# huj31415/nbody3d-webgpu

Hardware: AMD Instinct MI355X
Metric: pair-interactions/s (higher is better)
Workload: dtype f32; 1 GPU; N=262144 Plummer sphere, dt=1e-3, G=1, eps2=1e-4, i-sharded over 1 GPU(s); n=262144, kernel_variant=f32pk_symw_ipl16_j1_w2048_r32t128, parallelism=1gpu

## Files before the change

include/nbody3d_hip.h:

```cpp
#ifndef NBODY3D_HIP_H
#define NBODY3D_HIP_H

#include <stddef.h>
#include <stdint.h>

#ifdef __cplusplus
extern "C" {
#endif
#if defined(__GNUC__)
#pragma GCC visibility push(default)
#endif

#define NB_ABI_VERSION 2u
#define NB_ABI_MINOR 4u

typedef struct nb_sim nb_sim;

typedef enum nb_status {
    NB_OK = 0,
    NB_ERR_INVALID = 1,
    NB_ERR_NO_DEVICE = 2,
    NB_ERR_HIP = 3,
    NB_ERR_STATE = 4,
    NB_ERR_NOMEM = 5,
    NB_ERR_COMM = 6,
    NB_NOT_READY = 7
} nb_status;

typedef enum nb_precision { NB_F32 = 0, NB_F64 = 1 } nb_precision;

#define NB_FLAG_EXT_STREAM 1u
#define NB_FLAG_LDS_ONLY 4u
#define NB_FLAG_NO_FUSE 8u
#define NB_FLAG_POISON 16u

#define NB_FLAG_JPK_FENCED 32u

#define NB_FLAG_NO_SYM 64u

#define NB_FLAG_SYM_SHARD 128u

#define NB_FLAG_WHOLE_SWEEPS 256u

#define NB_FLAG_SINGLE_SWEEPS 512u

typedef enum nb_array { NB_BODIES = 0, NB_VEL = 1, NB_ACCEL = 2, NB_JERK = 3  } nb_array;

typedef enum nb_integrator { NB_INT_LEAPFROG = 0, NB_INT_HERMITE4 = 1 } nb_integrator;

typedef struct nb_config {
    uint32_t struct_size;
    uint32_t n;
    uint32_t precision;
    uint32_t tile;
    double eps2;
    int32_t device;
    uint32_t shard_begin;
    uint32_t shard_count;
    void *ext_stream;
    void *ext_bodies;
    uint32_t force_variant;
    uint32_t jsplit;
    uint32_t flags;
    uint32_t layer_budget_mib;
    uint32_t integrator;
    uint32_t reserved[3];
} nb_config;

uint32_t nb_abi_version(void);
uint32_t nb_abi_minor(void);

int nb_device_count(void);

int nb_create(const nb_config *cfg, nb_sim **out);

void nb_destroy(nb_sim *s);

int nb_upload(nb_sim *s, const void *bodies, const void *vel, const void *accel);

int nb_set_params(nb_sim *s, double dt, double G);

int nb_step(nb_sim *s, uint32_t nsteps);

int nb_download(nb_sim *s, void *bodies, void *vel, void *accel);

int nb_sync(nb_sim *s);

const char *nb_last_error(nb_sim *s);


int nb_device_ptr(nb_sim *s, int which , void **out);

typedef int (*nb_exchange_fn)(void *user, void *bodies_dev, size_t elem_size,
                              uint32_t n, uint32_t shard_begin,
                              uint32_t shard_count, void *hip_stream);
int nb_set_exchange(nb_sim *s, nb_exchange_fn fn, void *user);

typedef int (*nb_exchange_wait_fn)(void *user, void *hip_stream);
int nb_set_exchange_overlapped(nb_sim *s, nb_exchange_fn begin, nb_exchange_wait_fn wait, void *user);

#define NB_RCCL_ID_BYTES 128
#define NB_RCCL_OVERLAP 1u
int nb_rccl_unique_id(void *id_out );
int nb_rccl_attach(nb_sim *s, const void *id, int nranks, int rank, uint32_t flags);
int nb_rccl_detach(nb_sim *s);
int nb_rccl_info(nb_sim *s, int *nranks, int *rank, int *rccl_version);

typedef struct nb_multi nb_multi;
int nb_multi_create(const nb_config *cfg, uint32_t n_shards, const int32_t *devices, nb_multi **out);
void nb_multi_destroy(nb_multi *m);
int nb_multi_upload(nb_multi *m, const void *bodies, const void *vel, const void *accel);
int nb_multi_set_params(nb_multi *m, double dt, double G);
int nb_multi_step(nb_multi *m, uint32_t nsteps);
int nb_multi_download(nb_multi *m, void *bodies, void *vel, void *accel);
int nb_multi_sync(nb_multi *m);
const char *nb_multi_last_error(nb_multi *m);
int nb_multi_diagnostics(nb_multi *m, double out[5]);
const char *nb_multi_variant_name(nb_multi *m);
typedef enum nb_multi_collective { NB_MULTI_PEER = 0, NB_MULTI_RCCL = 1, NB_MULTI_PEER_OVERLAP = 2 } nb_multi_collective;
int nb_multi_set_collective(nb_multi *m, int mode );
int nb_multi_collective_info(nb_multi *m, int *mode, int *nranks, int *rccl_version);


int nb_enable_timing(nb_sim *s, int on);
int nb_kernel_times(nb_sim *s, double *force_ms, double *integrate_ms,
                    uint32_t *launches);
int nb_step_times(nb_sim *s, double *force_ms, double *integrate_ms, double *exchange_ms,
                  uint32_t *launches);
typedef struct nb_step_timing {
    uint32_t struct_size;
    uint32_t launches;
    double force_ms;
    double sym_reduce_ms;
    double reduce_scatter_ms;
    double integrate_ms;
    double allgather_ms;
    double span_ms;
    uint32_t reduce_scatters;
    uint32_t allgathers;
} nb_step_timing;
int nb_step_times2(nb_sim *s, nb_step_timing *out);
int nb_integrate_pass(nb_sim *s, uint32_t reps, double *avg_ms);
int nb_force_pass(nb_sim *s, uint32_t reps, double *avg_ms);

const char *nb_variant_name(nb_sim *s);

int nb_shape_info(nb_sim *s, uint32_t *jsplit, uint32_t *j_per_split, uint32_t *own_split0,
                  uint32_t *own_splits);



int nb_download_jerk(nb_sim *s, void *jerk);

int nb_upload_derivs(nb_sim *s, const void *accel, const void *jerk);

#define NB_BLOCK_FROZEN 1u
typedef struct nb_block_steps {
    uint32_t struct_size;
    uint32_t max_level;
    uint32_t min_level;
    uint32_t flags;
    double   eta;
} nb_block_steps;
int nb_set_block_steps(nb_sim *s, const nb_block_steps *cfg );

struct nb_block_stats {
    uint32_t struct_size, enabled;
    uint64_t outer_steps, block_steps, body_steps;
    uint64_t clamped;
    uint32_t finest_level, reserved;
};
int nb_block_stats(nb_sim *s, struct nb_block_stats *out, int reset);
int nb_download_levels(nb_sim *s, uint8_t *levels );
int nb_upload_levels(nb_sim *s, const uint8_t *levels );

int nb_frame_request(nb_sim *s);
int nb_frame_acquire(nb_sim *s, int wait, const float **bodies, const float **speed,
                     uint64_t *step_index);


int nb_diagnostics(nb_sim *s, double out[5]);

#define NB_FIELD_AT_BODIES 1u
#define NB_FIELD_F64       2u
#define NB_FIELD_DEVICE    4u
typedef struct nb_field_request {
    uint32_t struct_size;
    uint32_t m;
    uint32_t flags;
    uint32_t first_body;
    const void *points;
    void *accel;
    void *phi;
} nb_field_request;
int nb_field_eval(nb_sim *s, const nb_field_request *req);
int nb_multi_field_eval(nb_multi *m, const nb_field_request *req);

#define NB_NBR_AT_BODIES 1u
#define NB_NBR_DEVICE    4u
typedef struct nb_neighbor_request {
    uint32_t struct_size;
    uint32_t m;
    uint32_t flags;
    uint32_t first_body;
    const void *points;
    const void *radii;
    double radius;
    uint32_t *index;
    void *dist2;
    uint32_t *count;
} nb_neighbor_request;
int nb_neighbors(nb_sim *s, const nb_neighbor_request *req);
int nb_multi_neighbors(nb_multi *m, const nb_neighbor_request *req);
int nb_neighbors_shape(nb_sim *s, uint32_t m, uint32_t *batch, uint32_t *chunks, uint32_t *j_per_chunk);

#if defined(__GNUC__)
#pragma GCC visibility pop
#endif
#ifdef __cplusplus
}
#endif
#endif
```

nbody3d-webgpu_amd/csrc/kernels/symmetric.hip.h:

```cpp
#pragma once

namespace nb {

template <typename T> struct SymRowT { T x, y, z; };
using SymRow = SymRowT<float>;

constexpr uint32_t kFlushSteps = 4096;

template <int NG>
__device__ __forceinline__ void flush_resident_sums(float (*hi)[64], const int lane, const bool flushed, nb_f2 (&ax)[NG], nb_f2 (&ay)[NG], nb_f2 (&az)[NG])
{
    if (flushed) {
#pragma unroll
        for (int c = 0; c < NG; ++c) {
            hi[6 * c + 0][lane] += ax[c].x; hi[6 * c + 1][lane] += ay[c].x; hi[6 * c + 2][lane] += az[c].x;
            hi[6 * c + 3][lane] += ax[c].y; hi[6 * c + 4][lane] += ay[c].y; hi[6 * c + 5][lane] += az[c].y;
        }
    } else {
#pragma unroll
        for (int c = 0; c < NG; ++c) {
            hi[6 * c + 0][lane] = ax[c].x; hi[6 * c + 1][lane] = ay[c].x; hi[6 * c + 2][lane] = az[c].x;
            hi[6 * c + 3][lane] = ax[c].y; hi[6 * c + 4][lane] = ay[c].y; hi[6 * c + 5][lane] = az[c].y;
        }
    }
// ... 90 lines not shown
#pragma unroll
                    for (int c = 0; c < 4; ++c) r[c] = r[c] * d2[c];
#pragma unroll
                    for (int c = 0; c < 4; ++c) r[c] = nb_f2{nb_rsq(r[c].x), nb_rsq(r[c].y)};
#pragma unroll
                    for (int c = 0; c < 4; ++c) si[c] = pm * r[c];
#pragma unroll
                    for (int c = 0; c < 4; ++c) sj[c] = mi[c0g + c] * r[c];
#pragma unroll
                    for (int c = 0; c < 4; ++c) ax[c0g + c] = __builtin_elementwise_fma(si[c], dx[c], ax[c0g + c]);
#pragma unroll
                    for (int c = 0; c < 4; ++c) ay[c0g + c] = __builtin_elementwise_fma(si[c], dy[c], ay[c0g + c]);
#pragma unroll
                    for (int c = 0; c < 4; ++c) az[c0g + c] = __builtin_elementwise_fma(si[c], dz[c], az[c0g + c]);
#pragma unroll
                    for (int c = 0; c < 4; ++c) bx[u] = __builtin_elementwise_fma(-sj[c], dx[c], bx[u]);
#pragma unroll
                    for (int c = 0; c < 4; ++c) by[u] = __builtin_elementwise_fma(-sj[c], dy[c], by[u]);
#pragma unroll
                    for (int c = 0; c < 4; ++c) bz[u] = __builtin_elementwise_fma(-sj[c], dz[c], bz[u]);
                }
            }
#pragma unroll
            for (int u = 0; u < J; ++u) {
                tx[u] = wave_rot1(tx[u]); ty[u] = wave_rot1(ty[u]); tz[u] = wave_rot1(tz[u]); tm[u] = wave_rot1(tm[u]);
                bx[u] = nb_f2{wave_rot1(bx[u].x), wave_rot1(bx[u].y)};
                by[u] = nb_f2{wave_rot1(by[u].x), wave_rot1(by[u].y)};
                bz[u] = nb_f2{wave_rot1(bz[u].x), wave_rot1(bz[u].y)};
            }
        }
        if (sym) {
            SymRow* out = partial + (size_t)(pl.t_layer0 + d) * pl.np + tstart + lane;
            if constexpr (WS == 1) {
#pragma unroll
                for (int u = 0; u < J; ++u) out[u * 64] = SymRow{bx[u].x + bx[u].y, by[u].x + by[u].y, bz[u].x + bz[u].y};
            } else {
                const int buf = done++ & 1;
#pragma unroll
                for (int u = 0; u < J; ++u) {
                    red[buf][w][3 * u + 0][lane] = bx[u].x + bx[u].y;
                    red[buf][w][3 * u + 1][lane] = by[u].x + by[u].y;
                    red[buf][w][3 * u + 2][lane] = bz[u].x + bz[u].y;
                }
                __syncthreads();
                if (w == done % WS) {
#pragma unroll
                    for (int u = 0; u < J; ++u) {
                        float sx = red[buf][0][3 * u + 0][lane], sy = red[buf][0][3 * u + 1][lane], sz = red[buf][0][3 * u + 2][lane];
#pragma unroll
                        for (int ww = 1; ww < WS; ++ww) { sx += red[buf][ww][3 * u + 0][lane]; sy += red[buf][ww][3 * u + 1][lane]; sz += red[buf][ww][3 * u + 2][lane]; }
                        out[u * 64] = SymRow{sx, sy, sz};
                    }
                }
            }
        }
    }
    SymRow* out = partial + (size_t)(pl.r_layer0 + q) * pl.np + (size_t)g * S + w * RB + lane;
#pragma unroll
    for (int c = 0; c < NG; ++c) {
        out[(2 * c) * 64] = SymRow{ax[c].x, ay[c].x, az[c].x};
        out[(2 * c + 1) * 64] = SymRow{ax[c].y, ay[c].y, az[c].y};
    }
}

struct SymWK { uint32_t np, nsb, W, total_hi, total_lo, n_hi, zc, ups, r_layer0, t_layer0; };
#define SYMW_PLAN_PARAMS const uint32_t W_, const uint32_t ups_, const uint32_t nsb_, const uint32_t zc_, const uint32_t r_layer0_, const uint32_t t_layer0_
typedef uint32_t nb_u4 __attribute__((ext_vector_type(4)));
template <int TAIL>
__device__ __forceinline__ void symw_record_and_tail(const uint32_t* rec_at, nb_u4& rec, uint32_t (&tail)[TAIL])
{
    static_assert(TAIL == 1 || TAIL == 4, "f32: eps2; f64: G, eps2");
    constexpr int kTailOffset = 4 * 8 + 6 * 4;
    if constexpr (TAIL == 1) {
        asm volatile("s_load_dwordx4 %0, %2, 0x0\n\ts_load_dword %1, %3, %4\n\ts_waitcnt lgkmcnt(0)"
                     : "=&s"(rec), "=&s"(tail[0]) : "s"(rec_at), "s"(__builtin_amdgcn_kernarg_segment_ptr()), "n"(kTailOffset) : "memory");
    } else {
        nb_u4 t;
        asm volatile("s_load_dwordx4 %0, %2, 0x0\n\ts_load_dwordx4 %1, %3, %4\n\ts_waitcnt lgkmcnt(0)"
                     : "=&s"(rec), "=&s"(t) : "s"(rec_at), "s"(__builtin_amdgcn_kernarg_segment_ptr()), "n"(kTailOffset) : "memory");
        tail[0] = t.x; tail[1] = t.y; tail[2] = t.z; tail[3] = t.w;
    }
}

__device__ __forceinline__ SymWK symw_plan_words(uint32_t S, uint32_t cps, uint32_t W, uint32_t ups, uint32_t nsb, uint32_t zc, uint32_t r_layer0, uint32_t t_layer0)
{
    const uint32_t H = (nsb - 1u) >> 1, n_hi = (nsb & 1u) ? 0u : nsb >> 1;
    const uint32_t total_lo = (H + 1u) * cps + zc, total_hi = total_lo + (n_hi ? cps : 0u);
    return SymWK{(nsb + (zc ? 1u : 0u)) * S, nsb, W, total_hi, total_lo, n_hi, zc, ups, r_layer0, t_layer0};
}

template <int NG, int J, bool PAIR>
__device__ __forceinline__ void symw_sweeps(const uint32_t* __restrict__ gtab, const float4* __restrict__ bodies, SymRow* __restrict__ partial, SymRow* __restrict__ spill,
                                            SYMW_PLAN_PARAMS, uint32_t* __restrict__ queue, const uint32_t npieces, const uint32_t pieces_off)
{
    static_assert(!PAIR || J == 1, "paired sweeps: one traveler per lane and sweep");
    constexpr uint32_t S = 128u * NG;
    constexpr int GW = NG < 4 ? NG : 4;
    constexpr uint32_t CH = 64u * J;
    constexpr uint32_t CPS = S / CH;
    const SymWK pl = symw_plan_words(S, CPS, W_, ups_, nsb_, zc_, r_layer0_, t_layer0_);
    const int lane = threadIdx.x & 63, wi = threadIdx.x >> 6;
    const uint32_t w = __builtin_amdgcn_readfirstlane(blockIdx.x * 4u + wi);
    const bool active = w < pl.W;
    NB_STAMP(0);
    __shared__ float red[4][6 * NG][64];
    __shared__ uint32_t fin[4];
    const uint32_t ups = pl.ups, ush = (uint32_t)__builtin_ctz(ups), ustep = 64u >> ush,
                   tab1 = 2u * (pl.np / S);
    nb_u4 rec;
    uint32_t tail[1];
    symw_record_and_tail(gtab + tab1 + 4u * (active ? w : 0u), rec, tail);
    const float eps2 = __builtin_bit_cast(float, tail[0]);
    const nb_f2 e2 = nb_f2{eps2, eps2};
    const uint32_t first_lo = pl.n_hi * pl.total_hi, first_z = first_lo + (pl.nsb - pl.n_hi) * pl.total_lo;
    const uint32_t slot = rec.w;
    NB_STAMP_LIGHT(1);
    bool first_part = true;

    auto run = [&](uint32_t u, const uint32_t uend, const uint32_t piece_layer) -> uint32_t {
        uint32_t gfin = ~0u;
        while (u < uend) {
            const uint32_t p = u >> ush;
            uint32_t g, k, total;
            if (p < first_lo) { g = p / pl.total_hi; k = p - g * pl.total_hi; total = pl.total_hi; }
            else if (p < first_z) { const uint32_t r = p - first_lo; g = pl.n_hi + r / pl.total_lo; k = r - (g - pl.n_hi) * pl.total_lo; total = pl.total_lo; }
            else { g = pl.nsb; k = p - first_z; total = pl.zc; }
            const uint32_t ring = g < pl.nsb ? total - CPS - pl.zc : 0u;
            const uint32_t both_end = g < pl.nsb ? ring + pl.zc : 0u;
            uint32_t ug_end = (p - k + total) * ups;
            if (ug_end > uend) ug_end = uend;

            nb_f2 xi[NG], yi[NG], zi[NG], mi[NG], ax[NG], ay[NG], az[NG];
            {
                const float4* rb = bodies + (size_t)g * S + lane;
#pragma unroll
                for (int c = 0; c < NG; ++c) {
                    const float4 b0 = ld4(rb + (2 * c) * 64), b1 = ld4(rb + (2 * c + 1) * 64);
                    xi[c] = nb_f2{b0.x, b1.x}; yi[c] = nb_f2{b0.y, b1.y}; zi[c] = nb_f2{b0.z, b1.z}; mi[c] = nb_f2{b0.w, b1.w};
                    ax[c] = nb_f2{0, 0}; ay[c] = nb_f2{0, 0}; az[c] = nb_f2{0, 0};
                }
            }
            uint32_t since = 0;
            bool flushed = false;
            while (u < ug_end) {
                const uint32_t q0 = u & (ups - 1u);
                bool pair = false;
                if constexpr (PAIR) pair = q0 == 0u && ug_end - u >= 2u * ups && k + 1u < both_end;
                uint32_t nun = ups - q0;
                if (nun > ug_end - u) nun = ug_end - u;
                const uint32_t s0 = q0 * ustep, s1 = s0 + nun * ustep;
                u += pair ? 2u * ups : nun;
                if (since >= kFlushSteps) {
                    flush_resident_sums<NG>(red[wi], lane, flushed, ax, ay, az);
                    flushed = true;
                    since = 0;
                }
                since += pair ? 128u : s1 - s0;
                const bool sym = k < both_end, zsweep = k >= ring && sym;
                const uint32_t d = k / CPS;
                uint32_t tb = g + 1 + d;
                if (tb >= pl.nsb) tb -= pl.nsb;
                const uint32_t tstart = k < ring ? tb * S + (k % CPS) * CH : zsweep ? pl.nsb * S + (k - ring) * CH : g * S + (k - both_end) * CH;
                const uint32_t zrow = g * pl.zc + (k - ring);
                ++k;
                if constexpr (PAIR) {
                    if (pair) {
                        const bool zsweep1 = k >= ring;
                        const uint32_t d1 = k / CPS;
                        uint32_t tb1 = g + 1 + d1;
                        if (tb1 >= pl.nsb) tb1 -= pl.nsb;
                        const uint32_t tstart1 = zsweep1 ? pl.nsb * S + (k - ring) * CH : tb1 * S + (k % CPS) * CH;
                        const uint32_t zrow1 = g * pl.zc + (k - ring);
                        ++k;
                        const float4 t0 = ld4(bodies + tstart + lane), t1 = ld4(bodies + tstart1 + lane);
                        nb_f2 tx = nb_f2{t0.x, t1.x}, ty = nb_f2{t0.y, t1.y}, tz = nb_f2{t0.z, t1.z}, tm = nb_f2{t0.w, t1.w};
                        float bx0 = 0, bx1 = 0, by0 = 0, by1 = 0, bz0 = 0, bz1 = 0;
                        if (first_part) NB_STAMP(2);
                        for (uint32_t st = 0; st < 64u; ++st) {
                            nb_f2 sx = nb_f2{0, 0}, sy = nb_f2{0, 0}, sz = nb_f2{0, 0};
#pragma unroll
                            for (int c0g = 0; c0g < NG; c0g += GW) {
#pragma unroll
                                for (int f = 0; f < 2; ++f) {
                                    nb_f2 dx[GW], dy[GW], dz[GW], d2[GW], r[GW], si[GW], sj[GW];
#pragma unroll
                                    for (int c = 0; c < GW; ++c) dx[c] = symw_sub(f, tx, xi[c0g + c]);
#pragma unroll
                                    for (int c = 0; c < GW; ++c) dy[c] = symw_sub(f, ty, yi[c0g + c]);
#pragma unroll
                                    for (int c = 0; c < GW; ++c) dz[c] = symw_sub(f, tz, zi[c0g + c]);
#pragma unroll
                                    for (int c = 0; c < GW; ++c) d2[c] = __builtin_elementwise_fma(dx[c], dx[c], e2);
#pragma unroll
                                    for (int c = 0; c < GW; ++c) d2[c] = __builtin_elementwise_fma(dy[c], dy[c], d2[c]);
#pragma unroll
                                    for (int c = 0; c < GW; ++c) d2[c] = __builtin_elementwise_fma(dz[c], dz[c], d2[c]);
#pragma unroll
                                    for (int c = 0; c < GW; ++c) r[c] = d2[c] * d2[c];
#pragma unroll
                                    for (int c = 0; c < GW; ++c) r[c] = r[c] * d2[c];
#pragma unroll
                                    for (int c = 0; c < GW; ++c) r[c] = nb_f2{nb_rsq(r[c].x), nb_rsq(r[c].y)};
#pragma unroll
                                    for (int c = 0; c < GW; ++c) si[c] = symw_mul(f, tm, r[c]);
#pragma unroll
                                    for (int c = 0; c < GW; ++c) sj[c] = mi[c0g + c] * r[c];
#pragma unroll
                                    for (int c = 0; c < GW; ++c) ax[c0g + c] = __builtin_elementwise_fma(si[c], dx[c], ax[c0g + c]);
#pragma unroll
                                    for (int c = 0; c < GW; ++c) ay[c0g + c] = __builtin_elementwise_fma(si[c], dy[c], ay[c0g + c]);
#pragma unroll
                                    for (int c = 0; c < GW; ++c) az[c0g + c] = __builtin_elementwise_fma(si[c], dz[c], az[c0g + c]);
#pragma unroll
                                    for (int c = 0; c < GW; ++c) sx = symw_fnma(f, sj[c], dx[c], sx);
#pragma unroll
                                    for (int c = 0; c < GW; ++c) sy = symw_fnma(f, sj[c], dy[c], sy);
#pragma unroll
                                    for (int c = 0; c < GW; ++c) sz = symw_fnma(f, sj[c], dz[c], sz);
                                }
                            }
                            tx = nb_f2{wave_rot1(tx.x), wave_rot1(tx.y)}; ty = nb_f2{wave_rot1(ty.x), wave_rot1(ty.y)};
                            tz = nb_f2{wave_rot1(tz.x), wave_rot1(tz.y)}; tm = nb_f2{wave_rot1(tm.x), wave_rot1(tm.y)};
                            wave_rot1_add(bx0, sx.x); wave_rot1_add(bx1, sx.y); wave_rot1_add(by0, sy.x); wave_rot1_add(by1, sy.y);
                            wave_rot1_add(bz0, sz.x); wave_rot1_add(bz1, sz.y);
                            __builtin_amdgcn_sched_barrier(0);
                        }
                        if (first_part) { NB_STAMP_LIGHT(3); first_part = false; }
                        const uint32_t home = ((uint32_t)lane + 1u) & 63u;
                        SymRow* out0 = (zsweep ? spill + (size_t)zrow * CH : partial + (size_t)(pl.t_layer0 + d) * pl.np + tstart) + home;
                        SymRow* out1 = (zsweep1 ? spill + (size_t)zrow1 * CH : partial + (size_t)(pl.t_layer0 + d1) * pl.np + tstart1) + home;
                        *out0 = SymRow{bx0, by0, bz0};
                        *out1 = SymRow{bx1, by1, bz1};
                        continue;
                    }
                }
                float tx[J], ty[J], tz[J], tm[J];
                nb_f2 bx[J], by[J], bz[J];
                const uint32_t src = ((uint32_t)lane - s0) & 63u;
#pragma unroll
                for (int uu = 0; uu < J; ++uu) {
                    const float4 t = ld4(bodies + tstart + uu * 64 + src);
                    tx[uu] = t.x; ty[uu] = t.y; tz[uu] = t.z; tm[uu] = t.w;
                    bx[uu] = nb_f2{0, 0}; by[uu] = nb_f2{0, 0}; bz[uu] = nb_f2{0, 0};
                }
                auto steps = [&](auto both) {
                    constexpr bool BOTH = decltype(both)::value;
                    for (uint32_t st = s0; st < s1; ++st) {
#pragma unroll
                        for (int uu = 0; uu < J; ++uu) {
                            const nb_f2 px = nb_f2{tx[uu], tx[uu]}, py = nb_f2{ty[uu], ty[uu]}, pz = nb_f2{tz[uu], tz[uu]}, pm = nb_f2{tm[uu], tm[uu]};
#pragma unroll
                            for (int c0g = 0; c0g < NG; c0g += GW) {
                                nb_f2 dx[GW], dy[GW], dz[GW], d2[GW], r[GW], si[GW], sj[GW];
#pragma unroll
                                for (int c = 0; c < GW; ++c) dx[c] = px - xi[c0g + c];
#pragma unroll
                                for (int c = 0; c < GW; ++c) dy[c] = py - yi[c0g + c];
#pragma unroll
                                for (int c = 0; c < GW; ++c) dz[c] = pz - zi[c0g + c];
#pragma unroll
                                for (int c = 0; c < GW; ++c) d2[c] = __builtin_elementwise_fma(dx[c], dx[c], e2);
#pragma unroll
                                for (int c = 0; c < GW; ++c) d2[c] = __builtin_elementwise_fma(dy[c], dy[c], d2[c]);
#pragma unroll
                                for (int c = 0; c < GW; ++c) d2[c] = __builtin_elementwise_fma(dz[c], dz[c], d2[c]);
#pragma unroll
                                for (int c = 0; c < GW; ++c) r[c] = d2[c] * d2[c];
#pragma unroll
                                for (int c = 0; c < GW; ++c) r[c] = r[c] * d2[c];
#pragma unroll
                                for (int c = 0; c < GW; ++c) r[c] = nb_f2{nb_rsq(r[c].x), nb_rsq(r[c].y)};
#pragma unroll
                                for (int c = 0; c < GW; ++c) si[c] = pm * r[c];
                                if constexpr (BOTH) {
#pragma unroll
                                    for (int c = 0; c < GW; ++c) sj[c] = mi[c0g + c] * r[c];
                                }
#pragma unroll
                                for (int c = 0; c < GW; ++c) ax[c0g + c] = __builtin_elementwise_fma(si[c], dx[c], ax[c0g + c]);
#pragma unroll
                                for (int c = 0; c < GW; ++c) ay[c0g + c] = __builtin_elementwise_fma(si[c], dy[c], ay[c0g + c]);
#pragma unroll
                                for (int c = 0; c < GW; ++c) az[c0g + c] = __builtin_elementwise_fma(si[c], dz[c], az[c0g + c]);
                                if constexpr (BOTH) {
#pragma unroll
                                    for (int c = 0; c < GW; ++c) bx[uu] = __builtin_elementwise_fma(-sj[c], dx[c], bx[uu]);
#pragma unroll
                                    for (int c = 0; c < GW; ++c) by[uu] = __builtin_elementwise_fma(-sj[c], dy[c], by[uu]);
#pragma unroll
                                    for (int c = 0; c < GW; ++c) bz[uu] = __builtin_elementwise_fma(-sj[c], dz[c], bz[uu]);
                                }
                            }
                        }
#pragma unroll
                        for (int uu = 0; uu < J; ++uu) {
                            tx[uu] = wave_rot1(tx[uu]); ty[uu] = wave_rot1(ty[uu]); tz[uu] = wave_rot1(tz[uu]); tm[uu] = wave_rot1(tm[uu]);
                            if constexpr (BOTH) {
                                bx[uu] = nb_f2{wave_rot1(bx[uu].x), wave_rot1(bx[uu].y)};
                                by[uu] = nb_f2{wave_rot1(by[uu].x), wave_rot1(by[uu].y)};
                                bz[uu] = nb_f2{wave_rot1(bz[uu].x), wave_rot1(bz[uu].y)};
                            }
                        }
                    }
                };
                if (first_part) NB_STAMP(2);
                if (sym) steps(std::true_type{}); else steps(std::false_type{});
                if (first_part) { NB_STAMP_LIGHT(3); first_part = false; }
                if (sym) {
                    SymRow* out = (s0 != 0 ? spill + (size_t)slot * CH : zsweep ? spill + (size_t)zrow * CH : partial + (size_t)(pl.t_layer0 + d) * pl.np + tstart)
                                  + (((uint32_t)lane - s1) & 63u);
#pragma unroll
                    for (int uu = 0; uu < J; ++uu) out[uu * 64] = SymRow{bx[uu].x + bx[uu].y, by[uu].x + by[uu].y, bz[uu].x + bz[uu].y};
                }
            }
            if (u >= uend && piece_layer != ~0u) {
                SymRow* out = partial + (size_t)(pl.r_layer0 + piece_layer) * pl.np + (size_t)g * S + lane;
#pragma unroll
                for (int c = 0; c < NG; ++c) {
                    if (flushed) {
                        ax[c].x += red[wi][6 * c + 0][lane]; ay[c].x += red[wi][6 * c + 1][lane]; az[c].x += red[wi][6 * c + 2][lane];
                        ax[c].y += red[wi][6 * c + 3][lane]; ay[c].y += red[wi][6 * c + 4][lane]; az[c].y += red[wi][6 * c + 5][lane];
                    }
                    out[(2 * c) * 64] = SymRow{ax[c].x, ay[c].x, az[c].x};
                    out[(2 * c + 1) * 64] = SymRow{ax[c].y, ay[c].y, az[c].y};
                }
                return g;
            }
            if (u >= uend) {
                gfin = g;
#pragma unroll
                for (int c = 0; c < NG; ++c) {
                    if (flushed) {
                        ax[c].x += red[wi][6 * c + 0][lane]; ay[c].x += red[wi][6 * c + 1][lane]; az[c].x += red[wi][6 * c + 2][lane];
                        ax[c].y += red[wi][6 * c + 3][lane]; ay[c].y += red[wi][6 * c + 4][lane]; az[c].y += red[wi][6 * c + 5][lane];
                    }
                    red[wi][6 * c + 0][lane] = ax[c].x; red[wi][6 * c + 1][lane] = ay[c].x; red[wi][6 * c + 2][lane] = az[c].x;
                    red[wi][6 * c + 3][lane] = ax[c].y; red[wi][6 * c + 4][lane] = ay[c].y; red[wi][6 * c + 5][lane] = az[c].y;
                }
                break;
            }
            SymRow* out = partial + (size_t)(pl.r_layer0 + gtab[2 * g + 1] - 1u) * pl.np + (size_t)g * S + lane;
#pragma unroll
            for (int c = 0; c < NG; ++c) {
                if (flushed) {
                    ax[c].x += red[wi][6 * c + 0][lane]; ay[c].x += red[wi][6 * c + 1][lane]; az[c].x += red[wi][6 * c + 2][lane];
                    ax[c].y += red[wi][6 * c + 3][lane]; ay[c].y += red[wi][6 * c + 4][lane]; az[c].y += red[wi][6 * c + 5][lane];
                }
                out[(2 * c) * 64] = SymRow{ax[c].x, ay[c].x, az[c].x};
                out[(2 * c + 1) * 64] = SymRow{ax[c].y, ay[c].y, az[c].y};
            }
        }
        return gfin;
    };
    const uint32_t gfin = run(active ? rec.x : 0u, active ? rec.y : 0u, ~0u);
    NB_STAMP_LIGHT(8);
    if (lane == 0) fin[wi] = gfin;
    __syncthreads();
    NB_STAMP_LIGHT(9);
    if (gfin != ~0u) {
        int members = 0, mine = 0;
#pragma unroll
        for (int j = 0; j < 4; ++j) {
            const bool same = fin[j] == gfin;
            members += same;
            mine += same && j < wi;
        }
        SymRow* out = partial + (size_t)(pl.r_layer0 + rec.z) * pl.np + (size_t)gfin * S + lane;
        for (int r = mine; r < 2 * NG; r += members) {
            float sx = 0.f, sy = 0.f, sz = 0.f;
#pragma unroll
            for (int j = 0; j < 4; ++j)
                if (fin[j] == gfin) { sx += red[j][3 * r + 0][lane]; sy += red[j][3 * r + 1][lane]; sz += red[j][3 * r + 2][lane]; }
            out[r * 64] = SymRow{sx, sy, sz};
        }
    }
    if (npieces) {
        for (;;) {
            uint32_t id = 0;
            if (lane == 0) id = __hip_atomic_fetch_add(queue, 1u, __ATOMIC_RELAXED, __HIP_MEMORY_SCOPE_AGENT);
            id = __builtin_amdgcn_readfirstlane(id);
            if (id >= npieces) break;
            const uint32_t pu = gtab[pieces_off + 2u * id], ll = gtab[pieces_off + 2u * id + 1u];
            (void)run(pu, pu + (ll >> 16), ll & 0xffffu);
        }
    }
    NB_STAMP(4);
}

#define SYMW_KERNEL_PARAMS const uint32_t* __restrict__ gtab, const float4* __restrict__ bodies, SymRow* __restrict__ partial, SymRow* __restrict__ spill, \
                           SYMW_PLAN_PARAMS, const float eps2_arg ,                       \
                           uint32_t* __restrict__ queue, const uint32_t npieces, const uint32_t pieces_off
#define SYMW_KERNEL_ARGS gtab, bodies, partial, spill, W_, ups_, nsb_, zc_, r_layer0_, t_layer0_, queue, npieces, pieces_off
template <int NG, int J>
__global__ __launch_bounds__(256) __attribute__((amdgpu_waves_per_eu(NG >= 4 ? 2 : 4, NG > 4 ? 2 : (NG < 4 ? 8 : 4))))
void nb_force_symw(SYMW_KERNEL_PARAMS)
{
    symw_sweeps<NG, J, false>(SYMW_KERNEL_ARGS);
}
template <int NG>
__global__ __launch_bounds__(256) __attribute__((amdgpu_waves_per_eu(2, NG > 4 ? 2 : 4)))
void nb_force_symw_pairs(SYMW_KERNEL_PARAMS)
{
    symw_sweeps<NG, 1, true>(SYMW_KERNEL_ARGS);
}

__device__ __forceinline__ double wave_rot1(double v)
{
    const long long b = __builtin_bit_cast(long long, v);
    const int lo = (int)(b & 0xffffffffll), hi = (int)(b >> 32);
    const unsigned rlo = (unsigned)__builtin_amdgcn_update_dpp(lo, lo, 0x13C, 0xF, 0xF, false);
    const unsigned rhi = (unsigned)__builtin_amdgcn_update_dpp(hi, hi, 0x13C, 0xF, 0xF, false);
    return __builtin_bit_cast(double, (long long)(((unsigned long long)rhi << 32) | rlo));
}

template <int IPL>
__global__ __launch_bounds__(256) __attribute__((amdgpu_waves_per_eu(2, 2)))
void nb_force_symw64(const uint32_t* __restrict__ gtab, const double4* __restrict__ bodies, SymRowT<double>* __restrict__ partial, SymRowT<double>* __restrict__ spill,
                     SYMW_PLAN_PARAMS, const double G_arg, const double eps2_arg ,
                     uint32_t* __restrict__ queue, const uint32_t npieces, const uint32_t pieces_off)
{
    constexpr uint32_t S = 64u * IPL, CH = 64u, CPS = S / CH;
    const SymWK pl = symw_plan_words(S, CPS, W_, ups_, nsb_, zc_, r_layer0_, t_layer0_);
    constexpr int GW = 4;
    const int lane = threadIdx.x & 63, wi = threadIdx.x >> 6;
    const uint32_t w = __builtin_amdgcn_readfirstlane(blockIdx.x * 4u + wi);
    const bool active = w < pl.W;
    __shared__ double red[4][3 * IPL][64];
    __shared__ uint32_t fin[4];
    const uint32_t ups = pl.ups, ush = (uint32_t)__builtin_ctz(ups), ustep = 64u >> ush,
                   tab1 = 2u * (pl.np / S);
    nb_u4 rec;
    uint32_t tail[4];
    symw_record_and_tail(gtab + tab1 + 4u * (active ? w : 0u), rec, tail);
    const double G = __builtin_bit_cast(double, (unsigned long long)tail[1] << 32 | tail[0]), eps2 = __builtin_bit_cast(double, (unsigned long long)tail[3] << 32 | tail[2]);
    const uint32_t first_lo = pl.n_hi * pl.total_hi, first_z = first_lo + (pl.nsb - pl.n_hi) * pl.total_lo;
    const uint32_t slot = rec.w;
    auto run = [&](uint32_t u, const uint32_t uend, const uint32_t piece_layer) -> uint32_t {
        uint32_t gfin = ~0u;
        while (u < uend) {
            const uint32_t p = u >> ush;
            uint32_t g, k, total;
            if (p < first_lo) { g = p / pl.total_hi; k = p - g * pl.total_hi; total = pl.total_hi; }
            else if (p < first_z) { const uint32_t r = p - first_lo; g = pl.n_hi + r / pl.total_lo; k = r - (g - pl.n_hi) * pl.total_lo; total = pl.total_lo; }
            else { g = pl.nsb; k = p - first_z; total = pl.zc; }
            const uint32_t ring = g < pl.nsb ? total - CPS - pl.zc : 0u, both_end = g < pl.nsb ? ring + pl.zc : 0u;
            uint32_t ug_end = (p - k + total) * ups;
            if (ug_end > uend) ug_end = uend;
            double xi[IPL], yi[IPL], zi[IPL], mi[IPL], ax[IPL], ay[IPL], az[IPL];
#pragma unroll
            for (int c = 0; c < IPL; ++c) {
                const double4 b = ld4(bodies + (size_t)g * S + c * 64 + lane);
                xi[c] = b.x; yi[c] = b.y; zi[c] = b.z; mi[c] = b.w * G;
                ax[c] = 0; ay[c] = 0; az[c] = 0;
            }
            while (u < ug_end) {
                const uint32_t q0 = u & (ups - 1u);
                uint32_t nun = ups - q0;
                if (nun > ug_end - u) nun = ug_end - u;
                const uint32_t s0 = q0 * ustep, s1 = s0 + nun * ustep;
                u += nun;
                const bool sym = k < both_end, zsweep = k >= ring && sym;
                const uint32_t d = k / CPS;
                uint32_t tb = g + 1 + d;
                if (tb >= pl.nsb) tb -= pl.nsb;
                const uint32_t tstart = k < ring ? tb * S + (k % CPS) * CH : zsweep ? pl.nsb * S + (k - ring) * CH : g * S + (k - both_end) * CH;
                const uint32_t zrow = g * pl.zc + (k - ring);
                ++k;
                const double4 t = ld4(bodies + tstart + (((uint32_t)lane - s0) & 63u));
                double tx = t.x, ty = t.y, tz = t.z, tm = t.w * G, bx = 0, by = 0, bz = 0;
                auto steps = [&](auto both) {
                    constexpr bool BOTH = decltype(both)::value;
                    for (uint32_t st = s0; st < s1; ++st) {
#pragma unroll
                        for (int c0g = 0; c0g < IPL; c0g += GW) {
                            double dx[GW], dy[GW], dz[GW], d2[GW], y[GW], uu[GW];
#pragma unroll
                            for (int c = 0; c < GW; ++c) dx[c] = tx - xi[c0g + c];
#pragma unroll
                            for (int c = 0; c < GW; ++c) dy[c] = ty - yi[c0g + c];
#pragma unroll
                            for (int c = 0; c < GW; ++c) dz[c] = tz - zi[c0g + c];
#pragma unroll
                            for (int c = 0; c < GW; ++c) d2[c] = nb_fma(dz[c], dz[c], nb_fma(dy[c], dy[c], nb_fma(dx[c], dx[c], eps2)));
#pragma unroll
                            for (int c = 0; c < GW; ++c) y[c] = __builtin_amdgcn_rsq(d2[c]);
#pragma unroll
// ... 536 lines not shown
```

nbody3d-webgpu_amd/csrc/nb_engine.hip:

```cpp
#include "nb_internal.h"
#include "nb_kernels.hip.h"
#include "../../include/nbody3d_hip_plan.h"

#include <hip/hip_ext.h>

#include <algorithm>
#include <cmath>
#include <cstdio>
#include <cstdlib>
#include <cstring>
#include <new>
#include <type_traits>

namespace {
thread_local std::string g_create_error = "";
}

namespace nbi {
int fail(nb_sim* s, int code, const std::string& msg)
{
    if (s) s->err = msg; else g_create_error = msg;
    return code;
}
void set_create_error(const std::string& msg) { g_create_error = msg; }
// ... 10 lines not shown
        if (e_ != hipSuccess)                                                                             \
            return fail((s), NB_ERR_HIP, std::string(#call) + ": " + hipGetErrorString(e_));              \
    } while (0)

using namespace nbp;

#define NB_LS_CASES(F, NG, TL, ls)                                      \
    switch (ls) {                                                        \
        case 1: return (const void*)&nb::F<NG, 1, TL>;                   \
        case 2: return (const void*)&nb::F<NG, 2, TL>;                   \
        case 4: return (const void*)&nb::F<NG, 4, TL>;                   \
        case 8: return (const void*)&nb::F<NG, 8, TL>;                   \
        case 16: return (const void*)&nb::F<NG, 16, TL>;                 \
        case 32: return (const void*)&nb::F<NG, 32, TL>;                 \
        case 64: return (const void*)&nb::F<NG, 64, TL>;                 \
        default: return nullptr;                                         \
    }
#define NB_LS_CASES_T4(F, NG, ls)                                       \
    switch (ls) {                                                        \
        case 16: return (const void*)&nb::F<NG, 16, 4>;                  \
        case 32: return (const void*)&nb::F<NG, 32, 4>;                  \
        case 64: return (const void*)&nb::F<NG, 64, 4>;                  \
        default: return nullptr;                                         \
    }
#define NB_LS_CASES_T8(F, NG, ls)                                       \
    switch (ls) {                                                        \
        case 32: return (const void*)&nb::F<NG, 32, 8>;                  \
        case 64: return (const void*)&nb::F<NG, 64, 8>;                  \
        default: return nullptr;                                         \
    }
#define NB_PK_TABLE(NAME, F)                                            \
    const void* NAME(int ng, int ls, int tl)                            \
    {                                                                    \
        if (tl == 8) {           \
            if (ng == 1) { NB_LS_CASES_T8(F, 1, ls) }                    \
            if (ng == 2) { NB_LS_CASES_T8(F, 2, ls) }                    \
            if (ng == 4) { NB_LS_CASES_T8(F, 4, ls) }                    \
        }                                                                \
        if (tl == 1) {                                                   \
            if (ng == 1) { NB_LS_CASES(F, 1, 1, ls) }                    \
            if (ng == 2) { NB_LS_CASES(F, 2, 1, ls) }                    \
            if (ng == 4) { NB_LS_CASES(F, 4, 1, ls) }                    \
        } else if (tl == 4) {                                            \
            if (ng == 1) { NB_LS_CASES_T4(F, 1, ls) }                    \
            if (ng == 2) { NB_LS_CASES_T4(F, 2, ls) }                    \
            if (ng == 4) { NB_LS_CASES_T4(F, 4, ls) }                    \
        }                                                                \
        return nullptr;                                                  \
    }
NB_PK_TABLE(pk_force_kernel, nb_force_pk)
NB_PK_TABLE(pk_fused_kernel, nb_step_fused)

template <typename T>
const void* scalar_kernel(int ipl, int ls)
{
    if (ls == 1) {
        if (ipl == 1) return (const void*)&nb::nb_force<T, 1, 1>;
        if (ipl == 2) return (const void*)&nb::nb_force<T, 2, 1>;
        if (ipl == 4) return (const void*)&nb::nb_force<T, 4, 1>;
        return nullptr;
    }
    if (ipl != 1) return nullptr;
    if (ls == 4) return (const void*)&nb::nb_force<T, 1, 4>;
    if (ls == 16) return (const void*)&nb::nb_force<T, 1, 16>;
    if (ls == 64) return (const void*)&nb::nb_force<T, 1, 64>;
    return nullptr;
}

const void* sgpr_kernel(int ipl, int ws)
{
    if (ipl == 4 && ws == 5) return (const void*)&nb::nb_force_pk_sgpr<2, 4, true>;
    if (ipl == 4) return ws == 4 ? (const void*)&nb::nb_force_pk_sgpr<2, 4> : (const void*)&nb::nb_force_pk_sgpr<2, 1>;
    if (ipl == 8 && ws == 5) return (const void*)&nb::nb_force_pk_sgpr<4, 4, true>;
    if (ipl == 8) return ws == 4 ? (const void*)&nb::nb_force_pk_sgpr<4, 4> : (const void*)&nb::nb_force_pk_sgpr<4, 1>;
    return nullptr;
}

const void* rank_kernel_of(bool f64, int ipl)
{
    if (f64) return ipl == 8 ? (const void*)&nb::nb_force_symw64_rank<8> : nullptr;
    return ipl == 16 ? (const void*)&nb::nb_force_symw_rank<8> : ipl == 8 ? (const void*)&nb::nb_force_symw_rank<4> : nullptr;
}

const void* kernel_of(bool f64, const Shape& sh, bool single_sweeps = false)
{
    switch (sh.kind) {
        case kScalar: return f64 ? scalar_kernel<double>(sh.ipl, sh.ls) : scalar_kernel<float>(sh.ipl, sh.ls);
        case kPkLds: return f64 || (sh.ipl & 1) ? nullptr : pk_force_kernel(sh.ipl / 2, sh.ls, sh.x);
        case kFused: return f64 || (sh.ipl & 1) ? nullptr : pk_fused_kernel(sh.ipl / 2, sh.ls, sh.x);
        case kPkSgpr: return f64 || sh.ls != 1 || !(sh.x == 1 || sh.x == 4 || sh.x == 5) ? nullptr : sgpr_kernel(sh.ipl, sh.x);
        case kDirect:
            if (f64 || sh.ipl != 2 || sh.ls != 64) return nullptr;
            return sh.x == 1 ? (const void*)&nb::nb_step_direct<16> : sh.x == 2 ? (const void*)&nb::nb_step_direct<32> : nullptr;
        case kSym:
            if (sh.ls != 1) return nullptr;
            if (f64) return sh.ipl == 8 && sh.x == 3 ? (const void*)&nb::nb_force_symw64<8> : nullptr;
            if (sh.x == 4) return sh.ipl == 8 ? (const void*)&nb::nb_force_sym<4, 4, 2> : nullptr;
            if (sh.ipl == 4) return sh.x == 3 ? (const void*)&nb::nb_force_symw<2, 1> : nullptr;
            if (sh.ipl == 8 && sh.x == 3) return single_sweeps ? (const void*)&nb::nb_force_symw<4, 1> : (const void*)&nb::nb_force_symw_pairs<4>;
            if (sh.ipl == 16 && sh.x == 3) return single_sweeps ? (const void*)&nb::nb_force_symw<8, 1> : (const void*)&nb::nb_force_symw_pairs<8>;
            if (sh.ipl == 8) return sh.x == 1 ? (const void*)&nb::nb_force_symw<4, 2> : nullptr;
            if (sh.ipl == 16) return sh.x == 1 ? (const void*)&nb::nb_force_symw<8, 2> : nullptr;
            return nullptr;
        case kJpk:
            if (f64 || sh.ipl != 1 || sh.ls != 1) return nullptr;
            return sh.x == 4 ? (const void*)&nb::nb_step_jpk<4> : sh.x == 8 ? (const void*)&nb::nb_step_jpk<8>
                   : sh.x == 6 ? (const void*)&nb::nb_step_jpk<16> : nullptr;
        default: return nullptr;
    }
}

void plan_handle(nb_sim* s, const nb_config& cfg, int n_cu, double clock_hz, double device_mem)
{
    PlanInput in;
    if (device_mem > 0) in.device_mem = device_mem;
    in.n = s->n; in.sb = s->sb; in.sc = s->sc; in.f64 = s->f64; in.cfg = cfg; in.n_cu = n_cu; in.clock_hz = clock_hz;
    if (!s->no_device)
        in.occupancy = [f64 = s->f64](const Shape& sh, int block) {
            int occ = 0;
            const void* fn = kernel_of(f64, sh);
            if (!fn || hipOccupancyMaxActiveBlocksPerMultiprocessor(&occ, fn, block, 0) != hipSuccess) { (void)hipGetLastError(); return 0; }
            return occ;
        };
    LaunchPlan p = plan_launch(in);
    s->ipl = p.ipl; s->ls = p.ls; s->ws = p.ws; s->tl = p.tl;
    s->packed = p.packed; s->sgpr = p.sgpr; s->fused = p.fused; s->direct = p.direct; s->jpk = p.jpk; s->swap_acc = p.swap_acc;
    s->jsplit = p.jsplit; s->j_per_split = p.j_per_split; s->junits = p.junits; s->own_split0 = p.own_split0; s->own_splits = p.own_splits;
    s->sym = p.sym; s->symw = p.symw; s->sym_rank = p.sym_rank;
    s->sym_np = p.sym_np; s->sym_layers = p.sym_layers; s->sym_g0 = p.sym_g0; s->sym_g1 = p.sym_g1;
    static_assert(sizeof(s->sym_plan) == sizeof(p.sym_plan), "nb_sim::sym_plan mirrors LaunchPlan::sym_plan");
    memcpy(s->sym_plan, p.sym_plan, sizeof s->sym_plan);
    static_assert(sizeof(s->sym_rank_plan) == sizeof(p.sym_rank_plan), "nb_sim::sym_rank_plan mirrors LaunchPlan::sym_rank_plan");
    memcpy(s->sym_rank_plan, p.sym_rank_plan, sizeof s->sym_rank_plan);
    s->sym_passes = std::move(p.sym_passes);
    s->sym_local = p.sym_local;
    s->sym_tab_host = std::move(p.sym_tab_host);
    s->sym_spill_rows = p.sym_spill_rows;
    s->sym_pieces = p.sym_pieces;
    s->variant = std::move(p.variant);
}

Shape shape_of(const nb_sim* s)
{
    if (s->sym) return {kSym, s->ipl, 1, s->ws};
    if (s->jpk) return {kJpk, 1, 1, s->ws};
    if (s->direct) return {kDirect, s->ipl, s->ls, s->tl};
    if (s->fused) return {kFused, s->ipl, s->ls, s->tl};
    if (s->sgpr) return {kPkSgpr, s->ipl, 1, s->ws};
    if (s->packed) return {kPkLds, s->ipl, s->ls, s->tl};
    return {kScalar, s->ipl, s->ls, 1};
}

size_t sym_layer_rows(const nb_sim* s) { return s->sym_rank ? (size_t)(s->sym_g1 - s->sym_g0) * ipb_of(shape_of(s)) : (size_t)s->sym_np; }

bool streams_gm(const nb_sim* s) { return !s->f64 && s->packed && !s->jpk; }
bool gm_active(const nb_sim* s) { return streams_gm(s) && (float)s->G != 1.0f; }
const void* jstream(const nb_sim* s, int k) { return gm_active(s) ? s->gm[k] : s->bodies[k]; }

int ensure_gm(nb_sim* s)
{
    if (!gm_active(s)) { s->gm_ok = false; return NB_OK; }
    const size_t bytes = (size_t)16 * (s->sym ? s->sym_np : s->n);
    for (int k = 0; k < (s->fused ? 2 : 1); ++k)
        if (!s->gm[k]) {
            NB_HIP(s, hipMalloc(&s->gm[k], bytes));
            if (s->sym) NB_HIP(s, hipMemsetAsync(s->gm[k], 0, bytes, s->stream));
        }
    if (s->gm_ok && s->gm_G == s->G) return NB_OK;
    const float4* b = (const float4*)s->bodies[s->cur];
    float4* g = (float4*)s->gm[s->cur];
    uint32_t n = s->n;
    float G = (float)s->G;
    void* args[] = {&b, &g, &n, &G};
    NB_HIP(s, hipLaunchKernel((const void*)&nb::nb_gm_pack<0>, dim3(ceil_div(n, nb::kBlock)), dim3(nb::kBlock), args, 0, s->stream));
    s->gm_ok = true; s->gm_G = s->G;
    return NB_OK;
}

void launch_kernel(const void* fn, dim3 grid, dim3 block, void** args, hipStream_t stream, hipEvent_t t0, hipEvent_t t1)
{
    if (t0 || t1) (void)hipExtLaunchKernel(fn, grid, block, args, 0, stream, t0, t1, 0);
    else (void)hipLaunchKernel(fn, grid, block, args, 0, stream);
}

template <typename T>
void launch_force(nb_sim* s, int part = 0, hipEvent_t t0 = nullptr, hipEvent_t t1 = nullptr)
{
    using V4 = typename nb::vec4<T>::type;
    const Shape sh = shape_of(s);
    if (s->sym_rank) {
        const nbp::LaunchPlan::SymPass& ps = s->sym_passes[s->sym_pass];
        nb::SymRankPlan rp;
        memcpy(&rp, ps.plan, sizeof rp);
        uint32_t w0 = part == 2 ? rp.WA : 0u, w1 = part == 1 ? rp.WA : rp.WA + rp.WB;
        if (w1 <= w0) return;
        const void* b = jstream(s, s->cur);
        void* p = s->partial;
        const uint32_t* tab = s->sym_tab + ps.tab_off;
        uint32_t n = s->n, k_lo = ps.k_lo, k_hi = ps.k_hi, d0 = ps.d0;
        void* sp = s->sym_spill;
        if (s->f64) {
            double G = s->G, e2 = s->eps2;
            void* args[] = {&b, &p, &tab, &rp, &n, &G, &e2, &w0, &w1, &sp, &k_lo, &k_hi, &d0};
            launch_kernel(rank_kernel_of(true, sh.ipl), dim3(ceil_div(w1 - w0, 4u)), dim3(256), args, s->stream, t0, t1);
        } else {
            float e2 = (float)s->eps2;
            void* args[] = {&b, &p, &tab, &rp, &n, &e2, &w0, &w1, &sp, &k_lo, &k_hi, &d0};
            launch_kernel(rank_kernel_of(false, sh.ipl), dim3(ceil_div(w1 - w0, 4u)), dim3(256), args, s->stream, t0, t1);
        }
        return;
    }
    if (s->symw) {
        nb::SymWPlan pl;
        memcpy(&pl, s->sym_plan, sizeof pl);
        const void* b = jstream(s, s->cur);
        void* p = s->partial;
        const uint32_t* tab = s->sym_tab;
        void* sp = s->sym_spill;
        uint32_t* queue = s->sym_queue;
        uint32_t npieces = s->sym_pieces, pieces_off = 2u * (pl.np / ipb_of(sh)) + 4u * pl.W;
        if (npieces) (void)hipMemsetAsync(queue, 0, sizeof(uint32_t), s->stream);
        if (s->f64) {
            double G = s->G, e2 = s->eps2;
            void* args[] = {&tab, &b, &p, &sp, &pl.W, &pl.ups, &pl.nsb, &pl.zc, &pl.r_layer0, &pl.t_layer0, &G, &e2, &queue, &npieces, &pieces_off};
            launch_kernel(kernel_of(true, sh), dim3(ceil_div(pl.W, 4u)), dim3(256), args, s->stream, t0, t1);
        } else {
            float e2 = (float)s->eps2;
            void* args[] = {&tab, &b, &p, &sp, &pl.W, &pl.ups, &pl.nsb, &pl.zc, &pl.r_layer0, &pl.t_layer0, &e2, &queue, &npieces, &pieces_off};
            launch_kernel(kernel_of(false, sh, s->single_sweeps), dim3(ceil_div(pl.W, 4u)), dim3(256), args, s->stream, t0, t1);
        }
        return;
    }
    if (s->sym) {
        nb::SymPlan pl;
        memcpy(&pl, s->sym_plan, sizeof pl);
        const float4* b = (const float4*)jstream(s, s->cur);
        nb::SymRow* p = (nb::SymRow*)s->partial;
        float e2 = (float)s->eps2;
        uint32_t n = s->n;
        void* args[] = {&b, &p, &pl, &n, &e2};
        launch_kernel(kernel_of(false, sh), dim3(pl.nsb * pl.q), dim3(64 * sh.x), args, s->stream, t0, t1);
        return;
    }
    nb::SplitWindow win{0, 0xffffffffu, 0};
    uint32_t ny = s->jsplit;
    if (part == 1) { win.base = s->own_split0; ny = s->own_splits; }
    else if (part == 2) { win.hole_begin = s->own_split0; win.hole_count = s->own_splits; ny = s->jsplit - s->own_splits; }
    if (ny == 0) return;
    dim3 grid(ceil_div(s->sc, ipb_of(sh)), ny), block(nb::kBlock);
    const V4* b = (const V4*)jstream(s, s->cur);
    V4* p = (V4*)s->partial;
    T G = (T)s->G, e2 = (T)s->eps2;
    uint32_t n = s->n, sb = s->sb, sc = s->sc, jps = s->j_per_split;
    const V4* zr = (const V4*)s->zero_row;
    void* args[] = {&b, &p, &n, &sb, &sc, &G, &e2, &jps, &win, &zr};
    launch_kernel(kernel_of(s->f64, sh), grid, block, args, s->stream, t0, t1);
}

void ensure_pairs(nb_sim* s)
{
    if (!s->jpk || (s->pairs_ok && s->pairs_G == s->G)) return;
    const float4* b = (const float4*)s->bodies[s->cur];
    float4* p = (float4*)s->pairs[s->cur];
    uint32_t n = s->n;
    float G = (float)s->G;
    void* args[] = {&b, &p, &n, &G};
    (void)hipLaunchKernel((const void*)&nb::nb_pairs_pack<0>, dim3(ceil_div(ceil_div(n, 2u), nb::kBlock)), dim3(nb::kBlock), args, 0, s->stream);
    s->pairs_ok = true; s->pairs_G = s->G;
}

void launch_jpk(nb_sim* s, hipEvent_t t0, hipEvent_t t1)
{
    const Shape sh = shape_of(s);
    dim3 grid(ceil_div(s->n, 64u), s->jsplit), block(64 * jpk_ws(sh.x));
    const float4 *bin = (const float4*)s->bodies[s->cur], *pin = (const float4*)s->pairs[s->cur];
    float4 *bout = (float4*)s->bodies[s->cur ^ 1], *pout = (float4*)s->pairs[s->cur ^ 1];
    float4 *v = (float4*)s->vel, *a = (float4*)s->acc, *part = (float4*)s->jpartial;
    uint32_t* tk = s->tickets;
    uint32_t n = s->n, upw = s->junits, poison = (s->poison ? 1u : 0u) | (s->jpk_fenced ? 2u : 0u);
    float G = (float)s->G, e2 = (float)s->eps2, dt = (float)s->dt;
    void* args[] = {&bin, &pin, &bout, &pout, &v, &a, &part, &tk, &n, &upw, &poison, &G, &e2, &dt};
    launch_kernel(kernel_of(false, sh), grid, block, args, s->stream, t0, t1);
    s->cur ^= 1;
}

void launch_fused(nb_sim* s, hipEvent_t t0 = nullptr, hipEvent_t t1 = nullptr)
{
    if (s->jpk) { ensure_pairs(s); launch_jpk(s, t0, t1); return; }
    const Shape sh = shape_of(s);
    dim3 grid(ceil_div(s->n, ipb_of(sh))), block(nb::kBlock);
    const float4 *bin = (const float4*)s->bodies[s->cur], *jin = (const float4*)jstream(s, s->cur);
    float4 *bout = (float4*)s->bodies[s->cur ^ 1], *gout = gm_active(s) ? (float4*)s->gm[s->cur ^ 1] : nullptr;
    float4 *v = (float4*)s->vel, *a = (float4*)s->acc;
    uint32_t n = s->n;
    float G = (float)s->G, e2 = (float)s->eps2, dt = (float)s->dt;
    const float4* zr = (const float4*)s->zero_row;
    void* args[] = {&bin, &jin, &bout, &gout, &v, &a, &n, &G, &e2, &dt, &zr};
    launch_kernel(kernel_of(false, sh), grid, block, args, s->stream, t0, t1);
    s->cur ^= 1;
}

template <typename T>
void launch_integrate(nb_sim* s, hipEvent_t t0 = nullptr, hipEvent_t t1 = nullptr)
{
    using V4 = typename nb::vec4<T>::type;
    V4 *b = (V4*)s->bodies[s->cur], *v = (V4*)s->vel;
    uint32_t sb = s->sb, sc = s->sc, js = s->jsplit;
    T dt = (T)s->dt, G = (T)s->G;
    V4* gout = gm_active(s) && !(s->xfn || s->rccl) ? (V4*)s->gm[s->cur] : nullptr;
    if (s->sym_rank) {
        V4* a = (V4*)s->acc;
        const V4* p = (const V4*)s->sym_A + sb;
        uint32_t one = 1;
        V4* none = nullptr;
        void* args[] = {&b, &v, &a, &p, &sb, &sc, &one, &dt, &none, &G};
        launch_kernel((const void*)&nb::nb_integrate<T, 1>, dim3(ceil_div(sc, nb::kBlock)), dim3(nb::kBlock), args, s->stream, t0, t1);
        return;
    }
    if (s->symw) {
        nb::SymWPlan pl;
        memcpy(&pl, s->sym_plan, sizeof pl);
        V4* aa = (V4*)s->acc;
        const nb::SymRowT<T>* pp = (const nb::SymRowT<T>*)s->partial;
        const uint32_t* tab = s->sym_tab;
        uint32_t n = s->n, S = ipb_of(shape_of(s)), ch_shift = s->ws == 3 ? 6u : 7u;
        uint32_t shifts = (uint32_t)__builtin_ctz(S) | ch_shift << 8;
        uint32_t spill_off = pl.ups > 1 ? 2u * (pl.np / S) + 4u * pl.W : 0u;
        const void* sp = s->sym_spill;
        void* args[] = {&tab, &pp, &b, &v, &aa, &n, &shifts, &pl.np, &spill_off, &sp, &gout, &dt, &G, &pl.t_layer0, &pl.r_layer0, &pl.nsb, &pl.n_hi, &pl.H, &pl.zc};
        launch_kernel((const void*)&nb::nb_integrate_symw<T, 8>, dim3(ceil_div(n * 8u, nb::kBlock)), dim3(nb::kBlock), args, s->stream, t0, t1);
        return;
    }
    if (s->sym) {
        if constexpr (std::is_same<T, float>::value) {
            nb::SymPlan pl;
            memcpy(&pl, s->sym_plan, sizeof pl);
            float4 *bb = (float4*)b, *vv = (float4*)v, *aa = (float4*)s->acc, *gg = (float4*)gout;
            const nb::SymRow* pp = (const nb::SymRow*)s->partial;
            uint32_t n = s->n, S = ipb_of(shape_of(s));
            float fdt = (float)s->dt, fG = (float)s->G;
            void* args[] = {&bb, &vv, &aa, &pp, &n, &pl, &S, &fdt, &gg, &fG};
            launch_kernel((const void*)&nb::nb_integrate_sym<8>, dim3(ceil_div(n * 8u, nb::kBlock)), dim3(nb::kBlock), args, s->stream, t0, t1);
        }
        return;
    }
    if (s->swap_acc) {
        const V4 *ao = (const V4*)s->acc, *an = (const V4*)s->partial;
        void* args[] = {&b, &v, &ao, &an, &sb, &sc, &dt, &gout, &G};
        launch_kernel((const void*)&nb::nb_integrate_swap<T>, dim3(ceil_div(sc, nb::kBlock)), dim3(nb::kBlock), args, s->stream, t0, t1);
        std::swap(s->acc, s->partial);
        s->acc_parity ^= 1;
        return;
    }
    const int R = js >= 32 ? 8 : js >= 8 ? 4 : 1;
    V4* a = (V4*)s->acc;
    const V4* p = (const V4*)s->partial;
    void* args[] = {&b, &v, &a, &p, &sb, &sc, &js, &dt, &gout, &G};
    const void* fn = R == 8 ? (const void*)&nb::nb_integrate<T, 8> : R == 4 ? (const void*)&nb::nb_integrate<T, 4> : (const void*)&nb::nb_integrate<T, 1>;
    launch_kernel(fn, dim3(ceil_div(sc * (uint32_t)R, nb::kBlock)), dim3(nb::kBlock), args, s->stream, t0, t1);
}

void launch_step(nb_sim* s)
{
    if (s->fused) { launch_fused(s); return; }
    if (s->f64) { launch_force<double>(s); launch_integrate<double>(s); }
    else { launch_force<float>(s); launch_integrate<float>(s); }
}

constexpr uint32_t kGraphChunk = 16;
constexpr uint32_t kGraphBig = 128;
constexpr uint32_t kGraphSteps[2] = {kGraphChunk, kGraphBig};

void drop_graph(nb_sim* s)
{
    for (auto& g : s->graphs) {
        if (g.exec) { (void)hipGraphExecDestroy(g.exec); g.exec = nullptr; }
        if (g.graph) { (void)hipGraphDestroy(g.graph); g.graph = nullptr; }
    }
}

int role_parity(const nb_sim* s) { return s->cur | (s->acc_parity << 1); }

bool ensure_graph(nb_sim* s, int which)
{
    auto& slot = s->graphs[which];
    if (slot.exec && slot.dt == s->dt && slot.G == s->G && slot.parity == role_parity(s)) return true;
    if (slot.exec) { (void)hipGraphExecDestroy(slot.exec); slot.exec = nullptr; }
    if (slot.graph) { (void)hipGraphDestroy(slot.graph); slot.graph = nullptr; }
    void *acc0 = s->acc, *par0 = s->partial;
    const int cur0 = s->cur, par_bit0 = s->acc_parity;
    ensure_pairs(s);
    if (ensure_gm(s) != NB_OK) { s->graphs_ok = false; return false; }
    if (hipStreamBeginCapture(s->stream, hipStreamCaptureModeThreadLocal) != hipSuccess) { s->graphs_ok = false; return false; }
    for (uint32_t k = 0; k < kGraphSteps[which]; ++k) launch_step(s);
    hipGraph_t g = nullptr;
    const bool ok = hipStreamEndCapture(s->stream, &g) == hipSuccess && g;
    s->acc = acc0; s->partial = par0; s->cur = cur0; s->acc_parity = par_bit0;
    if (!ok) { (void)hipGetLastError(); s->graphs_ok = false; return false; }
    hipGraphExec_t ge = nullptr;
    if (hipGraphInstantiate(&ge, g, nullptr, nullptr, 0) != hipSuccess) { (void)hipGraphDestroy(g); (void)hipGetLastError(); s->graphs_ok = false; return false; }
    slot.graph = g; slot.exec = ge; slot.dt = s->dt; slot.G = s->G; slot.parity = role_parity(s);
    return true;
}

int finish_gather(nb_sim* s)
{
    if (!s->gather_pending) return NB_OK;
    s->gather_pending = false;
    if (s->rccl) return nbi::rccl_exchange_wait(s);
    if (!s->xwait) return NB_OK;
    const int rc = s->xwait(s->xuser, (void*)s->stream);
    if (rc != 0) return fail(s, NB_ERR_COMM, "exchange wait hook failed with code " + std::to_string(rc));
    return NB_OK;
}

int get_events(nb_sim* s, nb_events* out)
{
    if (s->pool_next == s->pool.size()) {
        if (s->pool.size() >= 4096) return 1;
        nb_events t;
        t.two = t.xchg = t.rs = t.blk = false;
        for (auto& e : t.e)
            if (hipEventCreate(&e) != hipSuccess) return 1;
        s->pool.push_back(t);
    }
    *out = s->pool[s->pool_next++];
    out->two = out->xchg = out->rs = out->blk = false;
    return 0;
}

void free_frames(nb_sim* s)
{
    for (auto& f : s->frame) {
        if (f.landed) (void)hipEventSynchronize(f.landed);
        if (f.h_bodies) (void)hipHostFree(f.h_bodies);
        if (f.d_bodies) (void)hipFree(f.d_bodies);
        if (f.packed) (void)hipEventDestroy(f.packed);
        if (f.landed) (void)hipEventDestroy(f.landed);
        f = nb_frame_slot();
    }
    if (s->frame_stream) { (void)hipStreamDestroy(s->frame_stream); s->frame_stream = nullptr; }
    s->frame_next = 0; s->frame_latest = -1;
}

constexpr uint32_t kFjWavesPerSimd = 8;
constexpr uint32_t kFjMinChunk = 2048;
constexpr uint32_t kFjMaxChunk = 1u << 20;

void fj_shape(uint32_t n, bool f64, int n_cu, uint32_t* chunks, uint32_t* per)
{
    const uint32_t rows = f64 ? nb::kFjRows64 : nb::kFjRows;
    const uint32_t want = kFjWavesPerSimd * (uint32_t)n_cu;
    uint32_t c = std::min(ceil_div(want, ceil_div(n, rows)), n / kFjMinChunk);
    c = std::max(std::max(c, 1u), ceil_div(n, kFjMaxChunk));
    *per = ceil_div(ceil_div(n, c), (uint32_t)nb::kTile) * nb::kTile;
    *chunks = ceil_div(n, *per);
}

void launch_fj(nb_sim* s, const void* pos, const void* vel, void* acc_out, void* jerk_out)
{
    uint32_t n = s->n, chunks = s->fj_chunks, per = s->fj_per;
    void* pa = s->fj_part;
    void* pj = (char*)s->fj_part + (size_t)4 * (s->f64 ? 8 : 4) * chunks * n;
    double G = s->G;
    void* rargs[] = {&pa, &pj, &n, &chunks, &G, &acc_out, &jerk_out};
    if (s->f64) {
        double e2 = s->eps2;
        void* args[] = {&pos, &vel, &pa, &pj, &n, &per, &e2};
        (void)hipLaunchKernel((const void*)&nb::nb_fj64<double>, dim3(ceil_div(n, nb::kFjRows64), chunks), dim3(nb::kBlock), args, 0, s->stream);
        (void)hipLaunchKernel((const void*)&nb::nb_fj_reduce<double, double>, dim3(ceil_div(n, nb::kBlock)), dim3(nb::kBlock), rargs, 0, s->stream);
    } else {
        float e2 = (float)s->eps2;
        const void* zr = s->zero_row;
        void* args[] = {&pos, &vel, &pa, &pj, &n, &per, &e2, &zr};
        (void)hipLaunchKernel((const void*)&nb::nb_fj_pk<nb::kFjNG>, dim3(ceil_div(n, nb::kFjRows), chunks), dim3(nb::kBlock), args, 0, s->stream);
        (void)hipLaunchKernel((const void*)&nb::nb_fj_reduce<float, float>, dim3(ceil_div(n, nb::kBlock)), dim3(nb::kBlock), rargs, 0, s->stream);
    }
}

int ensure_derivs(nb_sim* s, const char* who)
{
    if (!s->params_set) return fail(s, NB_ERR_STATE, std::string(who) + ": nb_set_params has not been called (G)");
    if (s->derivs_ok && s->derivs_any_G) { s->derivs_any_G = false; s->derivs_G = s->G; }
    if (s->derivs_ok && s->derivs_G == s->G) return NB_OK;
// ... 248 lines not shown
}

int nb_create(const nb_config* cfg_in, nb_sim** out)
{
    if (out) *out = nullptr;
    if (!cfg_in || !out) return fail(nullptr, NB_ERR_INVALID, "nb_create: null argument");
    nb_config cfg;
    uint32_t sb, sc;
    double eps2;
    if (const int rc = read_config(cfg_in, "nb_create", &cfg, &sb, &sc, &eps2)) return rc;

    int count = 0;
    hipError_t e = hipGetDeviceCount(&count);
    if (e != hipSuccess || count <= 0)
        return fail(nullptr, NB_ERR_NO_DEVICE,
                    std::string("nb_create: no HIP device (") + (e != hipSuccess ? hipGetErrorString(e) : "count = 0") +
                        "); this engine has no CPU fallback");
    int dev = cfg.device;
    if (dev < 0) { if (hipGetDevice(&dev) != hipSuccess) dev = 0; }
    if (dev >= count) return fail(nullptr, NB_ERR_INVALID, "nb_create: device ordinal out of range");

    nb_sim* s = new (std::nothrow) nb_sim;
    if (!s) return fail(nullptr, NB_ERR_NOMEM, "nb_create: out of host memory");
    s->n = cfg.n; s->sb = sb; s->sc = sc;
    s->f64 = cfg.precision == NB_F64;
    s->esz = s->f64 ? 8 : 4;
    s->eps2 = eps2;
    s->device = dev;

    auto bail = [&](int code, const std::string& msg) {
        std::string m = msg;
        nb_destroy(s);
        return fail(nullptr, code, m);
    };
#define NB_HIPC(call)                                                                        \
    do {                                                                                     \
        hipError_t e_ = (call);                                                              \
        if (e_ != hipSuccess) return bail(NB_ERR_HIP, std::string(#call) + ": " + hipGetErrorString(e_)); \
    } while (0)

    NB_HIPC(hipSetDevice(dev));
    hipDeviceProp_t prop;
    NB_HIPC(hipGetDeviceProperties(&prop, dev));
    if (cfg.ext_stream || (cfg.flags & NB_FLAG_EXT_STREAM)) { s->stream = (hipStream_t)cfg.ext_stream; s->own_stream = false; }
    else { NB_HIPC(hipStreamCreateWithFlags(&s->stream, hipStreamNonBlocking)); s->own_stream = true; }

    const int n_cu = prop.multiProcessorCount > 0 ? prop.multiProcessorCount : 256;
    s->n_cu = n_cu;
    const double clock_hz = prop.clockRate > 0 ? 1e3 * prop.clockRate : 2.4e9;
    if (cfg.integrator == NB_INT_HERMITE4) {
        s->hermite = true;
        fj_shape(s->n, s->f64, n_cu, &s->fj_chunks, &s->fj_per);
        s->jsplit = s->fj_chunks; s->j_per_split = s->fj_per;
        s->variant = std::string("hermite4_") + (s->f64 ? "f64" : "f32pk") + "_c" + std::to_string(s->fj_chunks) + "_j" + std::to_string(s->fj_per);
        const size_t hrow = 4 * s->esz;
        NB_HIPC(hipMalloc(&s->bodies[0], hrow * s->n));
        s->own_bodies = true;
        for (void** p : {&s->vel, &s->acc, &s->jerk, &s->hx, &s->hv}) NB_HIPC(hipMalloc(p, hrow * s->n));
        NB_HIPC(hipMalloc(&s->fj_part, (size_t)2 * hrow * s->fj_chunks * s->n));
        NB_HIPC(hipMalloc(&s->zero_row, 64));
        NB_HIPC(hipMemsetAsync(s->zero_row, 0, 64, s->stream));
        s->diag_chunk = nb::kTile * std::min(16u, std::max(1u, s->n / 16384u));
        s->diag_blocks = ceil_div(s->sc, nb::kDiagRows) * ceil_div(s->n, s->diag_chunk);
        NB_HIPC(hipMalloc((void**)&s->diag, sizeof(double) * 5 * s->diag_blocks));
        *out = s;
        return NB_OK;
    }
    plan_handle(s, cfg, n_cu, clock_hz, (double)prop.totalGlobalMem);
    if (s->sym && (!s->sym_rank || s->sym_local) && !cfg.force_variant) {
        size_t free_b = 0, total_b = 0;
        auto need = [&]() { return 3.0 * s->esz * (double)sym_layer_rows(s) * s->sym_layers + 12.0 * s->esz * s->sym_np; };
        if (hipMemGetInfo(&free_b, &total_b) == hipSuccess && need() > 0.9 * (double)free_b) {
            nb_config fit = cfg;
            fit.layer_budget_mib = (uint32_t)std::max(1.0, 0.6 * (double)free_b / 1048576.0);
            plan_handle(s, fit, n_cu, clock_hz, (double)prop.totalGlobalMem);
            if (s->sym && need() > 0.9 * (double)free_b) {
                cfg.flags |= NB_FLAG_NO_SYM;
                plan_handle(s, cfg, n_cu, clock_hz, (double)prop.totalGlobalMem);
            }
        }
    }
    if (!kernel_of(s->f64, shape_of(s))) return bail(NB_ERR_INVALID, "nb_create: no kernel for shape " + s->variant);
    s->single_sweeps = (cfg.flags & NB_FLAG_SINGLE_SWEEPS) != 0;

    const size_t row = 4 * s->esz;
    if (cfg.ext_bodies) { s->bodies[0] = cfg.ext_bodies; s->own_bodies = false; }
    else {
        const size_t rows = s->sym ? s->sym_np : s->n;
        NB_HIPC(hipMalloc(&s->bodies[0], row * rows));
        if (s->sym) NB_HIPC(hipMemset(s->bodies[0], 0, row * rows));
        s->own_bodies = true;
        if (s->fused) NB_HIPC(hipMalloc(&s->bodies[1], row * s->n));
    }
    NB_HIPC(hipMalloc(&s->vel, row * s->sc));
    NB_HIPC(hipMalloc(&s->acc, row * s->sc));
    auto alloc_partial = [&](size_t bytes) -> hipError_t {
        if (s->partial) return hipErrorInvalidValue;
        s->partial_bytes = bytes;
        return hipMalloc(&s->partial, bytes);
    };
    if (s->sym) {
        NB_HIPC(alloc_partial((size_t)3 * s->esz * sym_layer_rows(s) * s->sym_layers));
        if (s->sym_rank) NB_HIPC(hipMalloc(&s->sym_A, 4 * s->esz * s->sym_np));
        if (s->sym_spill_rows) {
            NB_HIPC(hipMalloc(&s->sym_spill, (size_t)3 * s->esz * s->sym_spill_rows));
            NB_HIPC(hipMemset(s->sym_spill, 0, (size_t)3 * s->esz * s->sym_spill_rows));
        }
        if (s->symw && s->sym_pieces) {
            NB_HIPC(hipMalloc((void**)&s->sym_queue, 64));
            NB_HIPC(hipMemset(s->sym_queue, 0, 64));
        }
        if (s->symw) {
            NB_HIPC(hipMalloc((void**)&s->sym_tab, sizeof(uint32_t) * s->sym_tab_host.size()));
            NB_HIPC(hipMemcpy(s->sym_tab, s->sym_tab_host.data(), sizeof(uint32_t) * s->sym_tab_host.size(), hipMemcpyHostToDevice));
        }
    } else if (!s->fused) {
        NB_HIPC(alloc_partial(row * s->sc * s->jsplit));
    }
    if (s->partial_bytes != (s->sym ? (size_t)3 * s->esz * sym_layer_rows(s) * s->sym_layers : s->fused ? (size_t)0 : row * s->sc * s->jsplit))
        return bail(NB_ERR_STATE, "nb_create: the partial-sum buffer does not have the size this handle's kernels index");
    if (s->jpk) {
        const size_t pbytes = ((size_t)ceil_div(ceil_div(s->n, 2u), 4u) + 3) * 128;
        const uint32_t iblocks = ceil_div(s->n, 64u);
        for (auto& p : s->pairs) { NB_HIPC(hipMalloc(&p, pbytes)); NB_HIPC(hipMemset(p, 0, pbytes)); }
        NB_HIPC(hipMalloc((void**)&s->tickets, sizeof(uint32_t) * iblocks));
        NB_HIPC(hipMemset(s->tickets, 0, sizeof(uint32_t) * iblocks));
        if (s->jsplit > 1) {
            NB_HIPC(hipMalloc(&s->jpartial, (size_t)16 * 64 * iblocks * s->jsplit));
            NB_HIPC(hipMemset(s->jpartial, 0xff, (size_t)16 * 64 * iblocks * s->jsplit));
        }
        NB_HIPC(hipDeviceSynchronize());
        s->poison = (cfg.flags & NB_FLAG_POISON) != 0;
        s->jpk_fenced = (cfg.flags & NB_FLAG_JPK_FENCED) != 0;
    }
    NB_HIPC(hipMalloc(&s->zero_row, 64));
    NB_HIPC(hipMemsetAsync(s->zero_row, 0, 64, s->stream));
    s->diag_chunk = nb::kTile * std::min(16u, std::max(1u, s->n / 16384u));
    s->diag_blocks = ceil_div(s->sc, nb::kDiagRows) * ceil_div(s->n, s->diag_chunk);
    NB_HIPC(hipMalloc((void**)&s->diag, sizeof(double) * 5 * s->diag_blocks));
#undef NB_HIPC
    *out = s;
    return NB_OK;
}

void nb_destroy(nb_sim* s)
{
    if (!s) return;
    (void)hipSetDevice(s->device);
    (void)finish_gather(s);
    if (s->stream) (void)hipStreamSynchronize(s->stream);
    nbi::rccl_release(s);
    drop_graph(s);
    free_frames(s);
    for (auto& t : s->pool)
        for (auto& e : t.e) (void)hipEventDestroy(e);
    if (s->own_bodies) {
        if (s->bodies[0]) (void)hipFree(s->bodies[0]);
        if (s->bodies[1]) (void)hipFree(s->bodies[1]);
    }
    if (s->vel) (void)hipFree(s->vel);
    if (s->acc) (void)hipFree(s->acc);
    if (s->partial) (void)hipFree(s->partial);
    for (auto& p : s->pairs) if (p) (void)hipFree(p);
    for (auto& p : s->gm) if (p) (void)hipFree(p);
    if (s->jpartial) (void)hipFree(s->jpartial);
    if (s->tickets) (void)hipFree(s->tickets);
    if (s->sym_tab) (void)hipFree(s->sym_tab);
    if (s->sym_spill) (void)hipFree(s->sym_spill);
    if (s->sym_queue) (void)hipFree(s->sym_queue);
    if (s->sym_A) (void)hipFree(s->sym_A);
    for (void* p : {s->jerk, s->hx, s->hv, s->fj_part, (void*)s->blk_lev, (void*)s->blk_due, (void*)s->blk_act, (void*)s->blk_hdr}) if (p) (void)hipFree(p);
    if (s->blk_hdr_host) (void)hipHostFree(s->blk_hdr_host);
    if (s->diag) (void)hipFree(s->diag);
    for (auto* b : {&s->fld_pts, &s->fld_acc, &s->fld_phi, &s->fld_part, &s->nbr_rad, &s->nbr_idx, &s->nbr_d2, &s->nbr_cnt, &s->nbr_inf})
        if (b->p) (void)hipFree(b->p);
    if (s->zero_row) (void)hipFree(s->zero_row);
    if (s->own_stream && s->stream) (void)hipStreamDestroy(s->stream);
    delete s;
}

const char* nb_last_error(nb_sim* s) { return s ? s->err.c_str() : g_create_error.c_str(); }

int nb_upload(nb_sim* s, const void* bodies, const void* vel, const void* accel)
{
    if (!s) return NB_ERR_INVALID;
    if (!bodies || !vel) return fail(s, NB_ERR_INVALID, "nb_upload: bodies and vel are required");
    NB_HIP(s, hipSetDevice(s->device));
    if (int rc = finish_gather(s)) return rc;
    const size_t row = 4 * s->esz;
    NB_HIP(s, hipStreamSynchronize(s->stream));
    NB_HIP(s, hipMemcpy(s->bodies[s->cur], bodies, row * s->n, hipMemcpyHostToDevice));
    NB_HIP(s, hipMemcpy(s->vel, (const char*)vel + row * s->sb, row * s->sc, hipMemcpyHostToDevice));
    if (s->hermite) {
        s->uploaded = true;
        s->derivs_ok = false;
        s->levels = 0;
        return NB_OK;
    }
    if (accel) NB_HIP(s, hipMemcpy(s->acc, (const char*)accel + row * s->sb, row * s->sc, hipMemcpyHostToDevice));
    else {
        NB_HIP(s, hipMemsetAsync(s->acc, 0, row * s->sc, s->stream));
        NB_HIP(s, hipStreamSynchronize(s->stream));
    }
    s->uploaded = true;
    s->pairs_ok = false;
    s->gm_ok = false;
    return NB_OK;
}

int nb_set_params(nb_sim* s, double dt, double G)
{
    if (!s) return NB_ERR_INVALID;
    if (!(dt == dt) || !(G == G)) return fail(s, NB_ERR_INVALID, "nb_set_params: NaN");
    if (s->params_set && (dt != s->dt || G != s->G)) s->levels = 0;
    s->dt = dt; s->G = G; s->params_set = true;
    return NB_OK;
}

int nb_step(nb_sim* s, uint32_t nsteps)
{
    if (!s) return NB_ERR_INVALID;
    if (!s->uploaded) return fail(s, NB_ERR_STATE, "nb_step: nb_upload has not been called");
    if (!s->params_set) return fail(s, NB_ERR_STATE, "nb_step: nb_set_params has not been called");
    if (!(s->dt > 0.0)) return NB_OK;
    NB_HIP(s, hipSetDevice(s->device));
    if (s->hermite) return s->blk ? block_step(s, nsteps) : hermite_step(s, nsteps);
    const bool exchange = s->xfn || s->rccl;
    ensure_pairs(s);
    if (gm_active(s) && !s->gm_ok) { if (int rc = finish_gather(s)) return rc; }
    if (int rc = ensure_gm(s)) return rc;
    if (s->own_stream && s->graphs_ok && !exchange && !s->timing && !s->sym_rank && nsteps >= kGraphChunk) {
        for (int which = 1; which >= 0; --which) {
            while (nsteps >= kGraphSteps[which] && ensure_graph(s, which)) {
                NB_HIP(s, hipGraphLaunch(s->graphs[which].exec, s->stream));
                nsteps -= kGraphSteps[which];
                s->steps_done += kGraphSteps[which];
            }
        }
    }
    for (uint32_t k = 0; k < nsteps; ++k) {
        if (exchange && gm_active(s) && !s->gm_ok) {
            if (int rc = finish_gather(s)) return rc;
            if (int rc = ensure_gm(s)) return rc;
        }
        if (s->sym_rank) {
            if (!s->rccl && !s->sym_local) return fail(s, NB_ERR_STATE, "nb_step: an NB_FLAG_SYM_SHARD handle needs nb_rccl_attach (or nb_multi) for its reduce-scatter");
            const bool split = s->gather_pending;
            if (!split) { if (int rc = finish_gather(s)) return rc; }
            nb_events evr;
            const bool recr = s->timing && get_events(s, &evr) == 0;
            if (recr) NB_HIP(s, hipEventRecord(evr.e[0], s->stream));
            if (int rc = nbi::sym_rank_phase_a(s, recr ? evr.e[7] : nullptr, split, recr && split ? &evr : nullptr)) return rc;
            if (recr) { NB_HIP(s, hipEventRecord(evr.e[1], s->stream)); evr.rs = true; }
            if (!s->sym_local) { if (int rc = nbi::rccl_reduce_scatter_A(s)) return rc; }
            if (recr) NB_HIP(s, hipEventRecord(evr.e[6], s->stream));
            if (int rc = nbi::sym_rank_phase_b(s)) return rc;
            if (recr) NB_HIP(s, hipEventRecord(evr.e[2], s->stream));
            NB_HIP(s, hipGetLastError());
            if (s->sym_local) { if (recr) s->pending.push_back(evr); continue; }
            if (int rc = nbi::rccl_exchange_begin(s)) return rc;
            if (nbi::rccl_overlapped(s)) s->gather_pending = true;
            else if (recr) { NB_HIP(s, hipEventRecord(evr.e[5], s->stream)); evr.xchg = true; }
            if (recr) s->pending.push_back(evr);
            continue;
        }
        nb_events ev;
        const bool rec = s->timing && get_events(s, &ev) == 0;
        hipEvent_t* e = rec ? ev.e : nullptr;
        if (s->fused) {
            launch_fused(s, e ? e[0] : nullptr, e ? e[1] : nullptr);
        } else {
            if (s->gather_pending) {
                if (s->f64) launch_force<double>(s, 1, e ? e[0] : nullptr, e ? e[1] : nullptr);
                else launch_force<float>(s, 1, e ? e[0] : nullptr, e ? e[1] : nullptr);
                if (int rc = finish_gather(s)) return rc;
                if (s->f64) launch_force<double>(s, 2, e ? e[3] : nullptr, e ? e[4] : nullptr);
                else launch_force<float>(s, 2, e ? e[3] : nullptr, e ? e[4] : nullptr);
                if (rec) ev.two = s->own_splits > 0 && s->own_splits < s->jsplit;
            } else {
                if (s->f64) launch_force<double>(s, 0, e ? e[0] : nullptr, e ? e[1] : nullptr);
                else launch_force<float>(s, 0, e ? e[0] : nullptr, e ? e[1] : nullptr);
            }
            if (s->f64) launch_integrate<double>(s, e ? e[6] : nullptr, e ? e[2] : nullptr);
            else launch_integrate<float>(s, e ? e[6] : nullptr, e ? e[2] : nullptr);
        }
        NB_HIP(s, hipGetLastError());
        ++s->steps_done;
        if (exchange) s->gm_ok = false;
        if (s->rccl) {
            if (int rc = nbi::rccl_exchange_begin(s)) return rc;
            if (nbi::rccl_overlapped(s)) {
                s->gather_pending = true;
                if (s->own_splits == 0) { if (int rc2 = finish_gather(s)) return rc2; }
            } else if (rec) {
                NB_HIP(s, hipEventRecord(ev.e[5], s->stream));
                ev.xchg = true;
            }
        } else if (s->xfn) {
            int rc = s->xfn(s->xuser, s->bodies[s->cur], s->esz, s->n, s->sb, s->sc, (void*)s->stream);
            if (rc != 0) return fail(s, NB_ERR_COMM, "nb_step: exchange hook failed with code " + std::to_string(rc));
            if (s->xwait) {
                s->gather_pending = true;
                if (s->own_splits == 0) { if (int rc2 = finish_gather(s)) return rc2; }
            }
        }
        if (rec) s->pending.push_back(ev);
    }
    return NB_OK;
}

int nb_sync(nb_sim* s)
{
    if (!s) return NB_ERR_INVALID;
    NB_HIP(s, hipSetDevice(s->device));
    if (int rc = finish_gather(s)) return rc;
    NB_HIP(s, hipStreamSynchronize(s->stream));
    return NB_OK;
}

int nb_download(nb_sim* s, void* bodies, void* vel, void* accel)
{
    if (!s) return NB_ERR_INVALID;
    if (!s->uploaded) return fail(s, NB_ERR_STATE, "nb_download: nothing uploaded yet");
    NB_HIP(s, hipSetDevice(s->device));
    if (int rc = finish_gather(s)) return rc;
    if (s->hermite && accel) { if (int rc = ensure_derivs(s, "nb_download")) return rc; }
    NB_HIP(s, hipStreamSynchronize(s->stream));
    const size_t row = 4 * s->esz;
    if (bodies) NB_HIP(s, hipMemcpy(bodies, s->bodies[s->cur], row * s->n, hipMemcpyDeviceToHost));
    if (vel) NB_HIP(s, hipMemcpy((char*)vel + row * s->sb, s->vel, row * s->sc, hipMemcpyDeviceToHost));
    if (accel) NB_HIP(s, hipMemcpy((char*)accel + row * s->sb, s->acc, row * s->sc, hipMemcpyDeviceToHost));
    return NB_OK;
}

int nb_device_ptr(nb_sim* s, int which, void** out)
{
    if (!s || !out) return NB_ERR_INVALID;
    if (which == NB_JERK && !s->hermite) return fail(s, NB_ERR_STATE, "nb_device_ptr: NB_JERK needs a Hermite handle (nb_config.integrator)");
    if (s->hermite && (which == NB_ACCEL || which == NB_JERK)) {
        if (!s->uploaded) return fail(s, NB_ERR_STATE, "nb_device_ptr: nothing uploaded yet");
        NB_HIP(s, hipSetDevice(s->device));
        if (int rc = ensure_derivs(s, "nb_device_ptr")) return rc;
    }
    switch (which) {
        case NB_BODIES: *out = s->bodies[s->cur]; s->pairs_ok = false; s->gm_ok = false; s->derivs_ok = false; s->levels = 0; break;
        case NB_VEL: *out = s->vel; s->derivs_ok = false; s->levels = 0; break;
        case NB_ACCEL: *out = s->acc; break;
        case NB_JERK: *out = s->jerk; break;
        default: return fail(s, NB_ERR_INVALID, "nb_device_ptr: unknown array");
    }
    return NB_OK;
}

int nb_download_jerk(nb_sim* s, void* jerk)
{
    if (!s) return fail(nullptr, NB_ERR_INVALID, "nb_download_jerk: null handle");
    if (!jerk) return fail(s, NB_ERR_INVALID, "nb_download_jerk: jerk is NULL");
    if (!s->hermite) return fail(s, NB_ERR_STATE, "nb_download_jerk: needs a Hermite handle (nb_config.integrator = NB_INT_HERMITE4)");
    if (!s->uploaded) return fail(s, NB_ERR_STATE, "nb_download_jerk: nothing uploaded yet");
    NB_HIP(s, hipSetDevice(s->device));
    if (int rc = ensure_derivs(s, "nb_download_jerk")) return rc;
    NB_HIP(s, hipStreamSynchronize(s->stream));
    NB_HIP(s, hipMemcpy(jerk, s->jerk, 4 * s->esz * s->n, hipMemcpyDeviceToHost));
    return NB_OK;
}

int nb_upload_derivs(nb_sim* s, const void* accel, const void* jerk)
{
    if (!s) return fail(nullptr, NB_ERR_INVALID, "nb_upload_derivs: null handle");
    if (!accel || !jerk) return fail(s, NB_ERR_INVALID, "nb_upload_derivs: accel and jerk are required");
    if (!s->hermite) return fail(s, NB_ERR_STATE, "nb_upload_derivs: needs a Hermite handle (nb_config.integrator = NB_INT_HERMITE4)");
    if (!s->uploaded) return fail(s, NB_ERR_STATE, "nb_upload_derivs: nb_upload has not been called");
    NB_HIP(s, hipSetDevice(s->device));
    NB_HIP(s, hipStreamSynchronize(s->stream));
    NB_HIP(s, hipMemcpy(s->acc, accel, 4 * s->esz * s->n, hipMemcpyHostToDevice));
    NB_HIP(s, hipMemcpy(s->jerk, jerk, 4 * s->esz * s->n, hipMemcpyHostToDevice));
    s->derivs_ok = true;
    s->derivs_any_G = !s->params_set;
    s->derivs_G = s->G;
    return NB_OK;
}

int nb_set_block_steps(nb_sim* s, const nb_block_steps* cfg)
{
    if (!s) return fail(nullptr, NB_ERR_INVALID, "nb_set_block_steps: null handle");
    if (!s->hermite) return fail(s, NB_ERR_STATE, "nb_set_block_steps: needs a Hermite handle (nb_config.integrator = NB_INT_HERMITE4)");
    if (!cfg) { s->blk = false; s->levels = 0; return NB_OK; }
    if (cfg->struct_size != sizeof(nb_block_steps)) return fail(s, NB_ERR_INVALID, "nb_set_block_steps: struct_size must be sizeof(nb_block_steps)");
    const uint32_t L = cfg->max_level ? cfg->max_level : 20u;
    if (cfg->max_level > 30) return fail(s, NB_ERR_INVALID, "nb_set_block_steps: max_level is at most 30");
    if (cfg->min_level > L) return fail(s, NB_ERR_INVALID, "nb_set_block_steps: min_level must not exceed max_level");
    if (cfg->flags & ~NB_BLOCK_FROZEN) return fail(s, NB_ERR_INVALID, "nb_set_block_steps: unknown flags");
    if (!(cfg->eta >= 0.0)) return fail(s, NB_ERR_INVALID, "nb_set_block_steps: eta must be > 0 (0: the default 0.02)");
    NB_HIP(s, hipSetDevice(s->device));
    if (!s->blk_lev) NB_HIP(s, hipMalloc((void**)&s->blk_lev, s->n));
    if (!s->blk_due) NB_HIP(s, hipMalloc((void**)&s->blk_due, sizeof(uint32_t) * s->n));
    if (!s->blk_act) NB_HIP(s, hipMalloc((void**)&s->blk_act, sizeof(uint32_t) * s->n));
    if (!s->blk_hdr) {
        NB_HIP(s, hipMalloc((void**)&s->blk_hdr, sizeof(uint32_t) * nb::kBlkWords));
        NB_HIP(s, hipMemsetAsync(s->blk_hdr, 0, sizeof(uint32_t) * nb::kBlkWords, s->stream));
    }
    if (!s->blk_hdr_host) NB_HIP(s, hipHostMalloc((void**)&s->blk_hdr_host, sizeof(uint32_t) * nb::kBlkWords, hipHostMallocDefault));
    if (!s->blk_hdr_pub) NB_HIP(s, hipHostGetDevicePointer((void**)&s->blk_hdr_pub, s->blk_hdr_host, 0));
    s->blk = true;
    s->blk_L = L; s->blk_lmin = cfg->min_level; s->blk_frozen = (cfg->flags & NB_BLOCK_FROZEN) != 0;
    s->blk_eta = cfg->eta > 0.0 ? cfg->eta : 0.02;
    s->levels = 0;
    return NB_OK;
}

int nb_block_stats(nb_sim* s, struct nb_block_stats* out, int reset)
{
    if (!s) return fail(nullptr, NB_ERR_INVALID, "nb_block_stats: null handle");
    if (!s->hermite) return fail(s, NB_ERR_STATE, "nb_block_stats: needs a Hermite handle (nb_config.integrator = NB_INT_HERMITE4)");
    if (!out || out->struct_size != sizeof(struct nb_block_stats)) return fail(s, NB_ERR_INVALID, "nb_block_stats: set out->struct_size to sizeof(nb_block_stats)");
    std::memset(out, 0, sizeof(*out));
    out->struct_size = sizeof(*out);
    out->enabled = s->blk ? 1u : 0u;
    if (!s->blk_hdr) return NB_OK;
    NB_HIP(s, hipSetDevice(s->device));
    uint32_t words[nb::kBlkWords];
    NB_HIP(s, hipStreamSynchronize(s->stream));
    NB_HIP(s, hipMemcpy(words, s->blk_hdr, sizeof words, hipMemcpyDeviceToHost));
    out->outer_steps = s->blk_outer; out->block_steps = s->blk_steps; out->body_steps = s->blk_body_steps;
    out->clamped = words[nb::kBlkClamped];
    out->finest_level = words[nb::kBlkFinest];
    if (reset) {
        s->blk_outer = s->blk_steps = s->blk_body_steps = 0;
        NB_HIP(s, hipMemsetAsync(s->blk_hdr, 0, sizeof(uint32_t) * nb::kBlkWords, s->stream));
    }
// ... 106 lines not shown
    t->integrate_ms = cnt ? g / cnt : 0.0;
    t->allgather_ms = nx ? x / nx : 0.0;
    t->span_ms = cnt ? span / cnt : 0.0;
    t->reduce_scatters = nrs;
    t->allgathers = nx;
    s->pending.clear();
    s->pool_next = 0;
    return NB_OK;
}

int nb_step_times2(nb_sim* s, nb_step_timing* out)
{
    if (!s) return NB_ERR_INVALID;
    if (!out || out->struct_size < sizeof(nb_step_timing)) return fail(s, NB_ERR_INVALID, "nb_step_times2: set out->struct_size to sizeof(nb_step_timing)");
    nb_step_timing t;
    memset(&t, 0, sizeof t);
    if (int rc = collect_times(s, &t)) return rc;
    t.struct_size = out->struct_size;
    memcpy(out, &t, sizeof t);
    return NB_OK;
}

int nb_step_times(nb_sim* s, double* force_ms, double* integrate_ms, double* exchange_ms, uint32_t* launches)
{
    if (!s) return NB_ERR_INVALID;
    nb_step_timing t;
    memset(&t, 0, sizeof t);
    if (int rc = collect_times(s, &t)) return rc;
    if (force_ms) *force_ms = t.force_ms + t.sym_reduce_ms;
    if (integrate_ms) *integrate_ms = t.integrate_ms;
    if (exchange_ms) *exchange_ms = t.reduce_scatter_ms + t.allgather_ms;
    if (launches) *launches = t.launches;
    return NB_OK;
}

int nb_kernel_times(nb_sim* s, double* force_ms, double* integrate_ms, uint32_t* launches)
{
    return nb_step_times(s, force_ms, integrate_ms, nullptr, launches);
}

int nb_integrate_pass(nb_sim* s, uint32_t reps, double* avg_ms)
{
    if (!s || !avg_ms) return NB_ERR_INVALID;
    if (!s->uploaded) return fail(s, NB_ERR_STATE, "nb_integrate_pass: nothing uploaded yet");
    if (s->hermite) return fail(s, NB_ERR_STATE, "nb_integrate_pass: a Hermite handle has no integrate kernel to run on its own (predictor and corrector belong to a step)");
    if (s->fused) return fail(s, NB_ERR_STATE, "nb_integrate_pass: a fused handle has no integrate kernel (create it with NB_FLAG_NO_FUSE)");
    if (reps == 0) return fail(s, NB_ERR_INVALID, "nb_integrate_pass: reps must be >= 1");
    NB_HIP(s, hipSetDevice(s->device));
    if (int rc = finish_gather(s)) return rc;
    const double dt = s->dt > 0 ? s->dt : 1e-3;
    const double keep = s->dt;
    s->dt = dt;
    if (s->steps_done == 0) {
        NB_HIP(s, hipMemsetAsync(s->partial, 0, s->sym ? (size_t)3 * s->esz * sym_layer_rows(s) * s->sym_layers : 4 * s->esz * s->sc * s->jsplit, s->stream));
        if (s->sym_rank) NB_HIP(s, hipMemsetAsync(s->sym_A, 0, 4 * s->esz * s->sym_np, s->stream));
    }
    hipEvent_t e0, e1;
    NB_HIP(s, hipEventCreate(&e0));
    NB_HIP(s, hipEventCreate(&e1));
    if (s->f64) launch_integrate<double>(s); else launch_integrate<float>(s);
    NB_HIP(s, hipEventRecord(e0, s->stream));
    for (uint32_t k = 0; k < reps; ++k) { if (s->f64) launch_integrate<double>(s); else launch_integrate<float>(s); }
    NB_HIP(s, hipEventRecord(e1, s->stream));
    NB_HIP(s, hipEventSynchronize(e1));
    float ms = 0;
    NB_HIP(s, hipEventElapsedTime(&ms, e0, e1));
    (void)hipEventDestroy(e0); (void)hipEventDestroy(e1);
    NB_HIP(s, hipGetLastError());
    s->dt = keep;
    drop_graph(s);
    *avg_ms = ms / reps;
    return NB_OK;
}

int nb_force_pass(nb_sim* s, uint32_t reps, double* avg_ms)
{
    if (!s || !avg_ms) return NB_ERR_INVALID;
    if (!s->uploaded) return fail(s, NB_ERR_STATE, "nb_force_pass: nothing uploaded yet");
    if (s->fused) return fail(s, NB_ERR_STATE, "nb_force_pass: a fused handle has no separate force kernel (create it with NB_FLAG_NO_FUSE)");
    if (reps == 0) return fail(s, NB_ERR_INVALID, "nb_force_pass: reps must be >= 1");
    NB_HIP(s, hipSetDevice(s->device));
    if (int rc = finish_gather(s)) return rc;
    if (int rc = ensure_gm(s)) return rc;
    if (s->hermite && !s->params_set) return fail(s, NB_ERR_STATE, "nb_force_pass: nb_set_params has not been called (G)");
    auto once = [&]() -> int {
        if (s->hermite) { launch_fj(s, s->bodies[0], s->vel, s->hx, s->hv); return NB_OK; }
        if (s->sym_rank) return s->f64 ? nbi::sym_rank_phase_a_t<double>(s, nullptr, false) : nbi::sym_rank_phase_a_t<float>(s, nullptr, false);
        if (s->f64) launch_force<double>(s); else launch_force<float>(s);
        return NB_OK;
    };
    hipEvent_t e0, e1;
    NB_HIP(s, hipEventCreate(&e0));
    NB_HIP(s, hipEventCreate(&e1));
    if (int rc = once()) return rc;
    NB_HIP(s, hipEventRecord(e0, s->stream));
    for (uint32_t k = 0; k < reps; ++k) { if (int rc = once()) return rc; }
    NB_HIP(s, hipEventRecord(e1, s->stream));
    NB_HIP(s, hipEventSynchronize(e1));
    float ms = 0;
    NB_HIP(s, hipEventElapsedTime(&ms, e0, e1));
    (void)hipEventDestroy(e0); (void)hipEventDestroy(e1);
    NB_HIP(s, hipGetLastError());
    *avg_ms = ms / reps;
    return NB_OK;
}

const char* nb_variant_name(nb_sim* s) { return s ? s->variant.c_str() : ""; }

int nb_shape_info(nb_sim* s, uint32_t* jsplit, uint32_t* j_per_split, uint32_t* own_split0, uint32_t* own_splits)
{
    if (!s) return NB_ERR_INVALID;
    if (jsplit) *jsplit = s->jsplit;
    if (j_per_split) *j_per_split = s->j_per_split;
    if (own_split0) *own_split0 = s->own_split0;
    if (own_splits) *own_splits = s->own_splits;
    return NB_OK;
}

int nb_plan_query(const nb_config* cfg_in, int n_cu, double clock_hz, nb_plan_info* out, uint32_t* tab, uint32_t tab_cap)
{
    if (!cfg_in || !out) return fail(nullptr, NB_ERR_INVALID, "nb_plan_query: null argument");
    if (out->struct_size < sizeof(nb_plan_info)) return fail(nullptr, NB_ERR_INVALID, "nb_plan_query: set out->struct_size to sizeof(nb_plan_info)");
    nb_config cfg;
    uint32_t sb, sc;
    double eps2;
    if (const int rc = read_config(cfg_in, "nb_plan_query", &cfg, &sb, &sc, &eps2)) return rc;
    if (cfg.integrator != NB_INT_LEAPFROG) return fail(nullptr, NB_ERR_INVALID, "nb_plan_query: integrator must be NB_INT_LEAPFROG (a Hermite handle has no launch plan: nb_shape_info reports its j-chunks)");
    int count = 0;
    double device_mem = 0.0;
    if (hipGetDeviceCount(&count) != hipSuccess) { (void)hipGetLastError(); count = 0; }
    if (n_cu <= 0 || !(clock_hz > 0)) {
        if (count <= 0) return fail(nullptr, NB_ERR_NO_DEVICE, "nb_plan_query: n_cu / clock_hz not given and there is no HIP device to read them from");
        int dev = cfg.device;
        if (dev < 0 && hipGetDevice(&dev) != hipSuccess) dev = 0;
        hipDeviceProp_t prop;
        if (dev >= count || hipSetDevice(dev) != hipSuccess || hipGetDeviceProperties(&prop, dev) != hipSuccess)
            return fail(nullptr, NB_ERR_HIP, "nb_plan_query: cannot read the device properties");
        if (n_cu <= 0) n_cu = prop.multiProcessorCount > 0 ? prop.multiProcessorCount : 256;
        if (!(clock_hz > 0)) clock_hz = prop.clockRate > 0 ? 1e3 * prop.clockRate : 2.4e9;
        device_mem = (double)prop.totalGlobalMem;
    }
    nb_sim tmp;
    tmp.n = cfg.n; tmp.sb = sb; tmp.sc = sc; tmp.f64 = cfg.precision == NB_F64; tmp.esz = tmp.f64 ? 8 : 4; tmp.eps2 = eps2;
    tmp.no_device = count <= 0;
    plan_handle(&tmp, cfg, n_cu, clock_hz, device_mem);
    const Shape sh = shape_of(&tmp);
    if (!kernel_of(tmp.f64, sh)) return fail(nullptr, NB_ERR_INVALID, "nb_plan_query: no kernel for shape " + tmp.variant);
    const uint32_t size = out->struct_size, want_pass = out->sym_pass;
    memset(out, 0, sizeof *out);
    out->struct_size = size;
    out->kind = (uint32_t)sh.kind; out->ipl = (uint32_t)sh.ipl; out->ls = (uint32_t)sh.ls; out->x = (uint32_t)sh.x;
    out->jsplit = tmp.jsplit; out->j_per_split = tmp.j_per_split; out->own_split0 = tmp.own_split0; out->own_splits = tmp.own_splits;
    out->sym = tmp.sym; out->symw = tmp.symw; out->sym_rank = tmp.sym_rank;
    out->sym_np = tmp.sym_np; out->sym_layers = tmp.sym_layers; out->sym_g0 = tmp.sym_g0; out->sym_g1 = tmp.sym_g1;
    static_assert(sizeof(out->sym_plan) == 11 * sizeof(uint32_t) && sizeof(tmp.sym_plan) >= 12 * sizeof(uint32_t), "nb_plan_info::sym_plan holds the first eleven words of nb_sim::sym_plan; the twelfth (ups) is sym_ups");
    memcpy(out->sym_plan, tmp.sym_plan, sizeof out->sym_plan);
    out->sym_ups = tmp.symw ? tmp.sym_plan[11] : 0;
    out->sym_spill_rows = tmp.sym_spill_rows;
    static_assert(sizeof(out->sym_rank_plan) == sizeof(tmp.sym_rank_plan), "nb_plan_info::sym_rank_plan mirrors nb_sim::sym_rank_plan");
    memcpy(out->sym_rank_plan, tmp.sym_rank_plan, sizeof out->sym_rank_plan);
    out->sym_passes = (uint32_t)tmp.sym_passes.size();
    out->sym_local = tmp.sym_local;
    size_t tab_from = 0, tab_to = tmp.sym_tab_host.size();
    if (!tmp.sym_passes.empty()) {
        if (want_pass >= tmp.sym_passes.size()) return fail(nullptr, NB_ERR_INVALID, "nb_plan_query: sym_pass out of range");
        const auto& ps = tmp.sym_passes[want_pass];
        out->sym_pass = want_pass;
        memcpy(out->sym_rank_plan, ps.plan, sizeof out->sym_rank_plan);
        out->sym_pass_k_lo = ps.k_lo; out->sym_pass_k_hi = ps.k_hi; out->sym_pass_d0 = ps.d0;
        tab_from = ps.tab_off;
        tab_to = want_pass + 1 < tmp.sym_passes.size() ? tmp.sym_passes[want_pass + 1].tab_off : tmp.sym_tab_host.size();
    }
    out->tab_len = (uint32_t)(tab_to - tab_from);
    snprintf(out->variant, sizeof out->variant, "%s", tmp.variant.c_str());
    if (tab) memcpy(tab, tmp.sym_tab_host.data() + tab_from, sizeof(uint32_t) * (out->tab_len < tab_cap ? out->tab_len : tab_cap));
    return NB_OK;
}

int nb_diagnostics(nb_sim* s, double out[5])
{
    if (!s || !out) return NB_ERR_INVALID;
    if (!s->uploaded) return fail(s, NB_ERR_STATE, "nb_diagnostics: nothing uploaded yet");
    NB_HIP(s, hipSetDevice(s->device));
    if (int rc = finish_gather(s)) return rc;
    dim3 grid(ceil_div(s->sc, nb::kDiagRows), ceil_div(s->n, s->diag_chunk)), block(nb::kBlock);
    if (s->f64)
        hipLaunchKernelGGL((nb::nb_diag<double>), grid, block, 0, s->stream, (const double4*)s->bodies[s->cur],
                           (const double4*)s->vel, s->n, s->sb, s->sc, s->diag_chunk, s->G, s->eps2, s->diag);
    else
        hipLaunchKernelGGL((nb::nb_diag<float>), grid, block, 0, s->stream, (const float4*)s->bodies[s->cur],
                           (const float4*)s->vel, s->n, s->sb, s->sc, s->diag_chunk, s->G, (float)s->eps2, s->diag);
    NB_HIP(s, hipGetLastError());
    std::vector<double> h((size_t)5 * s->diag_blocks);
    NB_HIP(s, hipMemcpyAsync(h.data(), s->diag, sizeof(double) * h.size(), hipMemcpyDeviceToHost, s->stream));
    NB_HIP(s, hipStreamSynchronize(s->stream));
    for (int q = 0; q < 5; ++q) out[q] = 0.0;
    for (uint32_t b = 0; b < s->diag_blocks; ++b)
        for (int q = 0; q < 5; ++q) out[q] += h[(size_t)b * 5 + q];
// ... 337 lines not shown
```

nbody3d-webgpu_amd/csrc/nb_internal.h:

```cpp
#pragma once
#include "../../include/nbody3d_hip.h"
#include "nb_plan.h"

#include <hip/hip_runtime.h>

#include <cstdint>
#include <string>
#include <vector>

struct nb_events { hipEvent_t e[8]; bool two, xchg, rs, blk; };

struct nb_rccl;

struct nb_frame_slot {
    float* h_bodies = nullptr;
    float* h_speed = nullptr;
    float* d_bodies = nullptr;
    float* d_speed = nullptr;
    hipEvent_t packed = nullptr;
    hipEvent_t landed = nullptr;
    uint64_t step = 0;
    bool in_flight = false, valid = false;
};

struct nb_sim {
    uint32_t n = 0, sb = 0, sc = 0;
    bool f64 = false;
    size_t esz = 4;
    int device = 0;
    bool no_device = false;
    double eps2 = 1e-4;
    hipStream_t stream = nullptr;
    bool own_stream = false;
    void* bodies[2] = {nullptr, nullptr};
    int cur = 0;
    bool own_bodies = false;
    void* gm[2] = {nullptr, nullptr};
    bool gm_ok = false;
    double gm_G = 0.0;
    void* vel = nullptr;
    void* acc = nullptr;
    void* partial = nullptr;
    size_t partial_bytes = 0;
    double* diag = nullptr;
    void* zero_row = nullptr;
    uint32_t diag_blocks = 0, diag_chunk = 256;
    double dt = 0.0, G = 0.0;
    bool params_set = false, uploaded = false;
    uint64_t steps_done = 0;
    int ipl = 1, ls = 1;
    bool packed = false;
    bool sgpr = false;
    int ws = 1;
    int tl = 1;
    bool fused = false;
    bool direct = false;
    bool jpk = false;
    void* pairs[2] = {nullptr, nullptr};
    bool pairs_ok = false;
    double pairs_G = 0.0;
    void* jpartial = nullptr;
    uint32_t* tickets = nullptr;
    uint32_t junits = 0;
    bool poison = false;
    bool jpk_fenced = false;
    int acc_parity = 0;
    bool swap_acc = false;
    uint32_t jsplit = 1, j_per_split = 0;
    bool sym = false;
    uint32_t sym_np = 0, sym_layers = 0;
    uint32_t sym_plan[16] = {0};
    bool symw = false;
    uint32_t* sym_tab = nullptr;
    std::vector<uint32_t> sym_tab_host;
    void* sym_spill = nullptr;
    uint32_t sym_spill_rows = 0;
    uint32_t sym_pieces = 0;
    bool single_sweeps = false;
    uint32_t* sym_queue = nullptr;
    bool sym_rank = false;
    uint32_t sym_g0 = 0, sym_g1 = 0;
    uint32_t sym_rank_plan[16] = {0};
    std::vector<nbp::LaunchPlan::SymPass> sym_passes;
    uint32_t sym_pass = 0;
    bool sym_local = false;
    void* sym_A = nullptr;
    std::string variant, err;
    nb_exchange_fn xfn = nullptr;
    nb_exchange_wait_fn xwait = nullptr;
    void* xuser = nullptr;
    bool gather_pending = false;
    uint32_t own_split0 = 0, own_splits = 0;
    nb_rccl* rccl = nullptr;
    bool timing = false;
    struct graph_slot {
        hipGraph_t graph = nullptr;
        hipGraphExec_t exec = nullptr;
        double dt = 0.0, G = 0.0;
        int parity = 0;
    } graphs[2];
    bool graphs_ok = true;
    std::vector<nb_events> pool;
    std::vector<nb_events> pending;
    size_t pool_next = 0;
    hipStream_t frame_stream = nullptr;
    static constexpr int kFrameSlots = 4;
    nb_frame_slot frame[kFrameSlots];
    int frame_next = 0;
    int frame_latest = -1;
    int n_cu = 256;
    struct field_buf { void* p = nullptr; size_t cap = 0; } fld_pts, fld_acc, fld_phi, fld_part;
    field_buf nbr_rad, nbr_idx, nbr_d2, nbr_cnt, nbr_inf;
    bool hermite = false;
    void* jerk = nullptr;
    void* hx = nullptr;
    void* hv = nullptr;
    void* fj_part = nullptr;
    uint32_t fj_chunks = 1, fj_per = 0;
    bool derivs_ok = false;
    bool derivs_any_G = false;
    double derivs_G = 0.0;
    bool blk = false, blk_frozen = false;
    uint32_t blk_L = 20, blk_lmin = 0;
    double blk_eta = 0.02;
    uint8_t* blk_lev = nullptr;
    uint32_t* blk_due = nullptr;
    uint32_t* blk_act = nullptr;
    uint32_t* blk_hdr = nullptr;
    uint32_t* blk_hdr_host = nullptr;
    uint32_t* blk_hdr_pub = nullptr;
    int levels = 0;
    uint64_t blk_outer = 0, blk_steps = 0, blk_body_steps = 0;
};

namespace nbi {

int fail(nb_sim* s, int code, const std::string& msg);
void set_create_error(const std::string& msg);
int neighbors(nb_sim* s, const nb_neighbor_request* req, uint32_t rows, const char* who);
const std::string& create_error();

int rccl_exchange_begin(nb_sim* s);
int rccl_reduce_scatter_A(nb_sim* s);
int sym_rank_phase_a(nb_sim* s, void* after_force = nullptr, bool split_at_gather = false, nb_events* stamps = nullptr);
int sym_rank_phase_b(nb_sim* s);
int rccl_exchange_wait(nb_sim* s);
bool rccl_overlapped(const nb_sim* s);
void rccl_release(nb_sim* s);

}
```

nbody3d-webgpu_amd/js/addon/nb_napi.c:

```c
#define NAPI_VERSION 6
#include <node_api.h>

#include <dlfcn.h>
#include <stdint.h>
#include <stdio.h>
#include <stdlib.h>
#include <string.h>

#include "../../../include/nbody3d_hip.h"
#include "../../../include/nbody3d_hip_plan.h"

static void *g_lib;
static uint32_t (*p_abi_version)(void);
static int (*p_device_count)(void);
static int (*p_create)(const nb_config *, nb_sim **);
static void (*p_destroy)(nb_sim *);
static int (*p_upload)(nb_sim *, const void *, const void *, const void *);
static int (*p_set_params)(nb_sim *, double, double);
static int (*p_step)(nb_sim *, uint32_t);
static int (*p_download)(nb_sim *, void *, void *, void *);
static int (*p_sync)(nb_sim *);
static const char *(*p_last_error)(nb_sim *);
static int (*p_enable_timing)(nb_sim *, int);
static int (*p_kernel_times)(nb_sim *, double *, double *, uint32_t *);
static const char *(*p_variant_name)(nb_sim *);
static int (*p_diagnostics)(nb_sim *, double *);
static int (*p_multi_create)(const nb_config *, uint32_t, const int32_t *, nb_multi **);
static void (*p_multi_destroy)(nb_multi *);
static int (*p_multi_upload)(nb_multi *, const void *, const void *, const void *);
static int (*p_multi_set_params)(nb_multi *, double, double);
static int (*p_multi_step)(nb_multi *, uint32_t);
static int (*p_multi_download)(nb_multi *, void *, void *, void *);
static int (*p_multi_sync)(nb_multi *);
static const char *(*p_multi_last_error)(nb_multi *);
static const char *(*p_multi_variant_name)(nb_multi *);
static int (*p_multi_diagnostics)(nb_multi *, double *);
static int (*p_multi_set_collective)(nb_multi *, int);
static int (*p_multi_collective_info)(nb_multi *, int *, int *, int *);
static int (*p_step_times)(nb_sim *, double *, double *, double *, uint32_t *);
static int (*p_step_times2)(nb_sim *, nb_step_timing *);
static int (*p_frame_request)(nb_sim *);
static int (*p_frame_acquire)(nb_sim *, int, const float **, const float **, uint64_t *);
static int (*p_plan_query)(const nb_config *, int, double, nb_plan_info *, uint32_t *, uint32_t);
static int (*p_field_eval)(nb_sim *, const nb_field_request *);
static int (*p_multi_field_eval)(nb_multi *, const nb_field_request *);
static int (*p_download_jerk)(nb_sim *, void *);
static int (*p_upload_derivs)(nb_sim *, const void *, const void *);
static int (*p_set_block_steps)(nb_sim *, const nb_block_steps *);
static int (*p_block_stats)(nb_sim *, struct nb_block_stats *, int);
static int (*p_download_levels)(nb_sim *, uint8_t *);
static int (*p_upload_levels)(nb_sim *, const uint8_t *);
static int (*p_neighbors)(nb_sim *, const nb_neighbor_request *);
static int (*p_multi_neighbors)(nb_multi *, const nb_neighbor_request *);

typedef struct { nb_sim *sim; nb_multi *multi; uint32_t n; int f64; } handle_t;

#define CHECK_NAPI(env, call)                                                        \
    do {                                                                             \
        if ((call) != napi_ok) {                                                     \
            napi_throw_error((env), NULL, "N-API call failed: " #call);              \
            return NULL;                                                             \
        }                                                                            \
    } while (0)

static napi_value throw_msg(napi_env env, int code, const char *msg, const char *where)
{
    char buf[768];
    snprintf(buf, sizeof buf, "%s: status %d: %s", where, code, msg ? msg : "");
    char codes[16];
    snprintf(codes, sizeof codes, "NB_%d", code);
    napi_throw_error(env, codes, buf);
    return NULL;
}

static napi_value throw_nb(napi_env env, int code, nb_sim *s, const char *where)
{
    char buf[768];
    const char *msg = p_last_error ? p_last_error(s) : "engine not loaded";
    snprintf(buf, sizeof buf, "%s: status %d: %s", where, code, msg ? msg : "");
    char codes[16];
    snprintf(codes, sizeof codes, "NB_%d", code);
    napi_throw_error(env, codes, buf);
    return NULL;
}

static int need_lib(napi_env env)
{
    if (!g_lib) { napi_throw_error(env, "NB_NOLIB", "libnbody3d_hip.so is not loaded; call load(path) first"); return 0; }
    return 1;
}

static napi_value undefined(napi_env env) { napi_value u; napi_get_undefined(env, &u); return u; }

static napi_value js_load(napi_env env, napi_callback_info info)
{
    size_t argc = 1; napi_value argv[1];
    CHECK_NAPI(env, napi_get_cb_info(env, info, &argc, argv, NULL, NULL));
    char path[4096]; size_t len = 0;
    if (argc < 1 || napi_get_value_string_utf8(env, argv[0], path, sizeof path, &len) != napi_ok) {
        napi_throw_type_error(env, NULL, "load(path): path string required"); return NULL;
    }
    if (!g_lib) {
        void *h = dlopen(path, RTLD_NOW | RTLD_LOCAL);
        if (!h) {
            char buf[4600]; snprintf(buf, sizeof buf, "cannot load HIP engine %s: %s", path, dlerror());
            napi_throw_error(env, "NB_NOLIB", buf); return NULL;
        }
#define SYM(var, name)                                                                            \
    do {                                                                                          \
        *(void **)(&var) = dlsym(h, name);                                                        \
        if (!var) { dlclose(h); napi_throw_error(env, "NB_NOLIB", "missing symbol " name); return NULL; } \
    } while (0)
        SYM(p_abi_version, "nb_abi_version"); SYM(p_device_count, "nb_device_count");
        SYM(p_create, "nb_create"); SYM(p_destroy, "nb_destroy"); SYM(p_upload, "nb_upload");
        SYM(p_set_params, "nb_set_params"); SYM(p_step, "nb_step"); SYM(p_download, "nb_download");
        SYM(p_sync, "nb_sync"); SYM(p_last_error, "nb_last_error"); SYM(p_enable_timing, "nb_enable_timing");
        SYM(p_kernel_times, "nb_kernel_times"); SYM(p_variant_name, "nb_variant_name");
        SYM(p_diagnostics, "nb_diagnostics");
        SYM(p_multi_create, "nb_multi_create"); SYM(p_multi_destroy, "nb_multi_destroy");
        SYM(p_multi_upload, "nb_multi_upload"); SYM(p_multi_set_params, "nb_multi_set_params");
        SYM(p_multi_step, "nb_multi_step"); SYM(p_multi_download, "nb_multi_download");
        SYM(p_multi_sync, "nb_multi_sync"); SYM(p_multi_last_error, "nb_multi_last_error");
        SYM(p_multi_variant_name, "nb_multi_variant_name"); SYM(p_multi_diagnostics, "nb_multi_diagnostics");
        SYM(p_multi_set_collective, "nb_multi_set_collective"); SYM(p_multi_collective_info, "nb_multi_collective_info");
        SYM(p_step_times, "nb_step_times"); SYM(p_step_times2, "nb_step_times2"); SYM(p_frame_request, "nb_frame_request"); SYM(p_frame_acquire, "nb_frame_acquire");
        SYM(p_plan_query, "nb_plan_query");
        SYM(p_field_eval, "nb_field_eval"); SYM(p_multi_field_eval, "nb_multi_field_eval");
#undef SYM
        *(void **)(&p_download_jerk) = dlsym(h, "nb_download_jerk");
        *(void **)(&p_upload_derivs) = dlsym(h, "nb_upload_derivs");
        *(void **)(&p_set_block_steps) = dlsym(h, "nb_set_block_steps");
        *(void **)(&p_block_stats) = dlsym(h, "nb_block_stats");
        *(void **)(&p_download_levels) = dlsym(h, "nb_download_levels");
        *(void **)(&p_upload_levels) = dlsym(h, "nb_upload_levels");
        *(void **)(&p_neighbors) = dlsym(h, "nb_neighbors");
        *(void **)(&p_multi_neighbors) = dlsym(h, "nb_multi_neighbors");
        g_lib = h;
    }
    if (p_abi_version() != NB_ABI_VERSION) { napi_throw_error(env, "NB_ABI", "ABI version mismatch"); return NULL; }
    napi_value v; CHECK_NAPI(env, napi_create_uint32(env, p_abi_version(), &v)); return v;
}

static napi_value js_device_count(napi_env env, napi_callback_info info)
{
    (void)info;
    if (!need_lib(env)) return NULL;
    napi_value v; CHECK_NAPI(env, napi_create_int32(env, p_device_count(), &v)); return v;
}

static void finalize_handle(napi_env env, void *data, void *hint)
{
    (void)env; (void)hint;
    handle_t *h = (handle_t *)data;
    if (h) {
        if (h->sim && p_destroy) p_destroy(h->sim);
        if (h->multi && p_multi_destroy) p_multi_destroy(h->multi);
        free(h);
    }
}

static int get_u32_prop(napi_env env, napi_value obj, const char *name, uint32_t *out)
{
    bool has = false; napi_value v;
    if (napi_has_named_property(env, obj, name, &has) != napi_ok || !has) return 0;
    if (napi_get_named_property(env, obj, name, &v) != napi_ok) return 0;
    napi_valuetype t; napi_typeof(env, v, &t);
    if (t != napi_number) return 0;
    double d; napi_get_value_double(env, v, &d);
    *out = (uint32_t)d; return 1;
}

static int get_f64_prop(napi_env env, napi_value obj, const char *name, double *out)
{
    bool has = false; napi_value v;
    if (napi_has_named_property(env, obj, name, &has) != napi_ok || !has) return 0;
    if (napi_get_named_property(env, obj, name, &v) != napi_ok) return 0;
    napi_valuetype t; napi_typeof(env, v, &t);
    if (t != napi_number) return 0;
    napi_get_value_double(env, v, out); return 1;
}

static void read_config(napi_env env, napi_value opts, nb_config *cfg)
{
    memset(cfg, 0, sizeof *cfg);
    cfg->struct_size = sizeof *cfg; cfg->device = -1;
    uint32_t u; double d;
    if (get_u32_prop(env, opts, "n", &u)) cfg->n = u;
    if (get_u32_prop(env, opts, "f64", &u)) cfg->precision = u ? NB_F64 : NB_F32;
    if (get_f64_prop(env, opts, "eps2", &d)) cfg->eps2 = d;
    if (get_f64_prop(env, opts, "device", &d)) cfg->device = (int32_t)d;
    if (get_u32_prop(env, opts, "shardBegin", &u)) cfg->shard_begin = u;
    if (get_u32_prop(env, opts, "shardCount", &u)) cfg->shard_count = u;
    if (get_u32_prop(env, opts, "variant", &u)) cfg->force_variant = u;
    if (get_u32_prop(env, opts, "jsplit", &u)) cfg->jsplit = u;
    if (get_u32_prop(env, opts, "tile", &u)) cfg->tile = u;
    if (get_u32_prop(env, opts, "flags", &u)) cfg->flags = u;
    if (get_u32_prop(env, opts, "layerBudgetMiB", &u)) cfg->layer_budget_mib = u;
    if (get_u32_prop(env, opts, "integrator", &u)) cfg->integrator = u;
}

static napi_value js_plan_query(napi_env env, napi_callback_info info)
{
    if (!need_lib(env)) return NULL;
    size_t argc = 1; napi_value argv[1];
    CHECK_NAPI(env, napi_get_cb_info(env, info, &argc, argv, NULL, NULL));
    if (argc < 1) { napi_throw_type_error(env, NULL, "planQuery(options) requires an object"); return NULL; }
    nb_config cfg; read_config(env, argv[0], &cfg);
    uint32_t n_cu = 0; double clock = 0.0;
    get_u32_prop(env, argv[0], "nCU", &n_cu);
    get_f64_prop(env, argv[0], "clockHz", &clock);
    nb_plan_info pi; memset(&pi, 0, sizeof pi); pi.struct_size = sizeof pi;
    int rc = p_plan_query(&cfg, (int)n_cu, clock, &pi, NULL, 0);
    if (rc != NB_OK) return throw_nb(env, rc, NULL, "nb_plan_query");
    napi_value o, v;
    CHECK_NAPI(env, napi_create_object(env, &o));
    CHECK_NAPI(env, napi_create_string_utf8(env, pi.variant, NAPI_AUTO_LENGTH, &v)); napi_set_named_property(env, o, "variant", v);
#define PUT_U32(name, val) do { napi_create_uint32(env, (val), &v); napi_set_named_property(env, o, name, v); } while (0)
    PUT_U32("kind", pi.kind); PUT_U32("ipl", pi.ipl); PUT_U32("ls", pi.ls); PUT_U32("x", pi.x);
    PUT_U32("jsplit", pi.jsplit); PUT_U32("jPerSplit", pi.j_per_split);
// ... 143 lines not shown
    if (argc < 4) { napi_throw_type_error(env, NULL, "download(handle, bodies|null, vel|null, accel|null)"); return NULL; }
    handle_t *h = get_handle(env, argv[0]); if (!h) return NULL;
    void *b, *v, *a;
    if (!get_array(env, argv[1], h, 1, &b, "bodies: typed array of 4*n elements or null")) return NULL;
    if (!get_array(env, argv[2], h, 1, &v, "vel: typed array of 4*n elements or null")) return NULL;
    if (!get_array(env, argv[3], h, 1, &a, "accel: typed array of 4*n elements or null")) return NULL;
    if (h->multi) {
        int rc = p_multi_download(h->multi, b, v, a);
        if (rc != NB_OK) return throw_msg(env, rc, p_multi_last_error(h->multi), "nb_multi_download");
        return undefined(env);
    }
    int rc = p_download(h->sim, b, v, a);
    if (rc != NB_OK) return throw_nb(env, rc, h->sim, "nb_download");
    return undefined(env);
}

static napi_value js_sync(napi_env env, napi_callback_info info)
{
    size_t argc = 1; napi_value argv[1];
    CHECK_NAPI(env, napi_get_cb_info(env, info, &argc, argv, NULL, NULL));
    handle_t *h = argc ? get_handle(env, argv[0]) : NULL; if (!h) return NULL;
    if (h->multi) {
        int rc = p_multi_sync(h->multi);
        if (rc != NB_OK) return throw_msg(env, rc, p_multi_last_error(h->multi), "nb_multi_sync");
        return undefined(env);
    }
    int rc = p_sync(h->sim);
    if (rc != NB_OK) return throw_nb(env, rc, h->sim, "nb_sync");
    return undefined(env);
}

static napi_value js_destroy(napi_env env, napi_callback_info info)
{
    size_t argc = 1; napi_value argv[1];
    CHECK_NAPI(env, napi_get_cb_info(env, info, &argc, argv, NULL, NULL));
    void *p = NULL;
    if (argc && napi_get_value_external(env, argv[0], &p) == napi_ok && p) {
        handle_t *h = (handle_t *)p;
        if (h->sim) { p_destroy(h->sim); h->sim = NULL; }
        if (h->multi) { p_multi_destroy(h->multi); h->multi = NULL; }
    }
    return undefined(env);
}

static napi_value js_enable_timing(napi_env env, napi_callback_info info)
{
    size_t argc = 2; napi_value argv[2];
    CHECK_NAPI(env, napi_get_cb_info(env, info, &argc, argv, NULL, NULL));
    handle_t *h = argc ? get_handle(env, argv[0]) : NULL; if (!h) return NULL;
    if (h->multi) { napi_throw_error(env, "NB_1", "per-kernel timing is not available on a multi-device handle"); return NULL; }
    bool on = true; if (argc >= 2) napi_get_value_bool(env, argv[1], &on);
    int rc = p_enable_timing(h->sim, on ? 1 : 0);
    if (rc != NB_OK) return throw_nb(env, rc, h->sim, "nb_enable_timing");
    return undefined(env);
}

static napi_value js_kernel_times(napi_env env, napi_callback_info info)
{
    size_t argc = 1; napi_value argv[1];
    CHECK_NAPI(env, napi_get_cb_info(env, info, &argc, argv, NULL, NULL));
    handle_t *h = argc ? get_handle(env, argv[0]) : NULL; if (!h) return NULL;
    if (h->multi) { napi_throw_error(env, "NB_1", "per-kernel timing is not available on a multi-device handle"); return NULL; }
    double f, g; uint32_t c;
    int rc = p_kernel_times(h->sim, &f, &g, &c);
    if (rc != NB_OK) return throw_nb(env, rc, h->sim, "nb_kernel_times");
    napi_value o, v;
    CHECK_NAPI(env, napi_create_object(env, &o));
    napi_create_double(env, f, &v); napi_set_named_property(env, o, "forceMs", v);
    napi_create_double(env, g, &v); napi_set_named_property(env, o, "integrateMs", v);
    napi_create_uint32(env, c, &v); napi_set_named_property(env, o, "launches", v);
    return o;
}

static napi_value js_variant(napi_env env, napi_callback_info info)
{
    size_t argc = 1; napi_value argv[1];
    CHECK_NAPI(env, napi_get_cb_info(env, info, &argc, argv, NULL, NULL));
    handle_t *h = argc ? get_handle(env, argv[0]) : NULL; if (!h) return NULL;
    napi_value v;
    CHECK_NAPI(env, napi_create_string_utf8(env, h->multi ? p_multi_variant_name(h->multi) : p_variant_name(h->sim), NAPI_AUTO_LENGTH, &v));
    return v;
}

static napi_value js_diagnostics(napi_env env, napi_callback_info info)
{
    size_t argc = 1; napi_value argv[1];
    CHECK_NAPI(env, napi_get_cb_info(env, info, &argc, argv, NULL, NULL));
    handle_t *h = argc ? get_handle(env, argv[0]) : NULL; if (!h) return NULL;
    double out[5];
    if (h->multi) {
        int rcm = p_multi_diagnostics(h->multi, out);
        if (rcm != NB_OK) return throw_msg(env, rcm, p_multi_last_error(h->multi), "nb_multi_diagnostics");
    } else {
        int rc = p_diagnostics(h->sim, out);
        if (rc != NB_OK) return throw_nb(env, rc, h->sim, "nb_diagnostics");
    }
    napi_value o, v, arr;
    CHECK_NAPI(env, napi_create_object(env, &o));
    napi_create_double(env, out[0], &v); napi_set_named_property(env, o, "kinetic", v);
    napi_create_double(env, out[1], &v); napi_set_named_property(env, o, "potential", v);
    napi_create_array_with_length(env, 3, &arr);
    for (uint32_t i = 0; i < 3; ++i) { napi_create_double(env, out[2 + i], &v); napi_set_element(env, arr, i, v); }
    napi_set_named_property(env, o, "momentum", arr);
    return o;
}


static napi_value js_step_times(napi_env env, napi_callback_info info)
{
    size_t argc = 1; napi_value argv[1];
    CHECK_NAPI(env, napi_get_cb_info(env, info, &argc, argv, NULL, NULL));
    handle_t *h = argc ? get_handle(env, argv[0]) : NULL; if (!h) return NULL;
    if (h->multi) { napi_throw_error(env, "NB_1", "per-kernel timing is not available on a multi-device handle"); return NULL; }
    nb_step_timing t;
    memset(&t, 0, sizeof t);
    t.struct_size = sizeof t;
    int rc = p_step_times2(h->sim, &t);
    if (rc != NB_OK) return throw_nb(env, rc, h->sim, "nb_step_times2");
    const double f = t.force_ms + t.sym_reduce_ms, g = t.integrate_ms, x = t.reduce_scatter_ms + t.allgather_ms;
    const uint32_t c = t.launches;
    napi_value o, v;
    CHECK_NAPI(env, napi_create_object(env, &o));
    napi_create_double(env, t.sym_reduce_ms, &v); napi_set_named_property(env, o, "symReduceMs", v);
    napi_create_double(env, t.reduce_scatter_ms, &v); napi_set_named_property(env, o, "reduceScatterMs", v);
    napi_create_double(env, t.allgather_ms, &v); napi_set_named_property(env, o, "allgatherMs", v);
    napi_create_double(env, t.span_ms, &v); napi_set_named_property(env, o, "spanMs", v);
    napi_create_double(env, f, &v); napi_set_named_property(env, o, "forceMs", v);
    napi_create_double(env, g, &v); napi_set_named_property(env, o, "integrateMs", v);
    napi_create_double(env, x, &v); napi_set_named_property(env, o, "exchangeMs", v);
    napi_create_uint32(env, c, &v); napi_set_named_property(env, o, "launches", v);
    return o;
}

static napi_value js_collective_info(napi_env env, napi_callback_info info)
{
    size_t argc = 1; napi_value argv[1];
    CHECK_NAPI(env, napi_get_cb_info(env, info, &argc, argv, NULL, NULL));
    handle_t *h = argc ? get_handle(env, argv[0]) : NULL; if (!h) return NULL;
    int mode = -1, nranks = 0, ver = 0;
    if (h->multi) {
        int rc = p_multi_collective_info(h->multi, &mode, &nranks, &ver);
        if (rc != NB_OK) return throw_msg(env, rc, p_multi_last_error(h->multi), "nb_multi_collective_info");
    }
    napi_value o, v;
    CHECK_NAPI(env, napi_create_object(env, &o));
    napi_create_string_utf8(env, mode == NB_MULTI_RCCL ? "rccl" : (mode == NB_MULTI_PEER ? "peer" : "none"), NAPI_AUTO_LENGTH, &v);
    napi_set_named_property(env, o, "mode", v);
    napi_create_int32(env, nranks, &v); napi_set_named_property(env, o, "nranks", v);
    napi_create_int32(env, ver, &v); napi_set_named_property(env, o, "rcclVersion", v);
    return o;
}

static napi_value js_request_frame(napi_env env, napi_callback_info info)
{
    size_t argc = 1; napi_value argv[1];
    CHECK_NAPI(env, napi_get_cb_info(env, info, &argc, argv, NULL, NULL));
    handle_t *h = argc ? get_handle(env, argv[0]) : NULL; if (!h) return NULL;
    if (h->multi) { napi_throw_error(env, "NB_1", "the frame feed is not available on a multi-device handle"); return NULL; }
    int rc = p_frame_request(h->sim);
    if (rc != NB_OK) return throw_nb(env, rc, h->sim, "nb_frame_request");
    return undefined(env);
}

static napi_value js_frame(napi_env env, napi_callback_info info)
{
    size_t argc = 4; napi_value argv[4];
// ... 171 lines not shown
        if (argc < 5) { napi_throw_type_error(env, NULL, "setBlockSteps(handle, eta, maxLevel, minLevel, frozen)"); return NULL; }
        nb_block_steps cfg;
        memset(&cfg, 0, sizeof cfg);
        cfg.struct_size = sizeof cfg;
        uint32_t u = 0; bool frozen = false;
        CHECK_NAPI(env, napi_get_value_double(env, argv[1], &cfg.eta));
        CHECK_NAPI(env, napi_get_value_uint32(env, argv[2], &u)); cfg.max_level = u;
        CHECK_NAPI(env, napi_get_value_uint32(env, argv[3], &u)); cfg.min_level = u;
        CHECK_NAPI(env, napi_get_value_bool(env, argv[4], &frozen));
        cfg.flags = frozen ? NB_BLOCK_FROZEN : 0u;
        rc = p_set_block_steps(h->sim, &cfg);
    }
    if (rc != NB_OK) return throw_nb(env, rc, h->sim, "nb_set_block_steps");
    return undefined(env);
}

static napi_value js_block_stats(napi_env env, napi_callback_info info)
{
    size_t argc = 2; napi_value argv[2];
    CHECK_NAPI(env, napi_get_cb_info(env, info, &argc, argv, NULL, NULL));
    if (argc < 1) { napi_throw_type_error(env, NULL, "blockStats(handle, reset)"); return NULL; }
    handle_t *h = block_handle(env, argv[0], *(void **)&p_block_stats, "nb_block_stats"); if (!h) return NULL;
    bool reset = false;
    if (argc > 1) napi_get_value_bool(env, argv[1], &reset);
    struct nb_block_stats st;
    memset(&st, 0, sizeof st);
    st.struct_size = sizeof st;
    int rc = p_block_stats(h->sim, &st, reset ? 1 : 0);
    if (rc != NB_OK) return throw_nb(env, rc, h->sim, "nb_block_stats");
    napi_value o, v;
    CHECK_NAPI(env, napi_create_object(env, &o));
    napi_get_boolean(env, st.enabled != 0, &v); napi_set_named_property(env, o, "enabled", v);
    napi_create_double(env, (double)st.outer_steps, &v); napi_set_named_property(env, o, "outerSteps", v);
    napi_create_double(env, (double)st.block_steps, &v); napi_set_named_property(env, o, "blockSteps", v);
    napi_create_double(env, (double)st.body_steps, &v); napi_set_named_property(env, o, "bodySteps", v);
    napi_create_double(env, (double)st.clamped, &v); napi_set_named_property(env, o, "clamped", v);
    napi_create_uint32(env, st.finest_level, &v); napi_set_named_property(env, o, "finestLevel", v);
    return o;
}

static int get_levels(napi_env env, napi_value v, const handle_t *h, uint8_t **out)
{
    bool is_ta = false; napi_is_typedarray(env, v, &is_ta);
    napi_typedarray_type tt = napi_int8_array; size_t len = 0; void *data = NULL; napi_value ab; size_t off;
    if (!is_ta || napi_get_typedarray_info(env, v, &tt, &len, &data, &ab, &off) != napi_ok || tt != napi_uint8_array) {
        napi_throw_type_error(env, NULL, "levels must be a Uint8Array of n elements"); return 0;
    }
    if (len != (size_t)h->n) { napi_throw_range_error(env, NULL, "levels must be a Uint8Array of n elements"); return 0; }
    *out = (uint8_t *)data; return 1;
}

static napi_value js_download_levels(napi_env env, napi_callback_info info)
{
    size_t argc = 2; napi_value argv[2];
    CHECK_NAPI(env, napi_get_cb_info(env, info, &argc, argv, NULL, NULL));
    if (argc < 2) { napi_throw_type_error(env, NULL, "downloadLevels(handle, levelsOut)"); return NULL; }
    handle_t *h = block_handle(env, argv[0], *(void **)&p_download_levels, "nb_download_levels"); if (!h) return NULL;
    uint8_t *lv;
    if (!get_levels(env, argv[1], h, &lv)) return NULL;
    int rc = p_download_levels(h->sim, lv);
    if (rc != NB_OK) return throw_nb(env, rc, h->sim, "nb_download_levels");
    return undefined(env);
}

static napi_value js_upload_levels(napi_env env, napi_callback_info info)
{
    size_t argc = 2; napi_value argv[2];
    CHECK_NAPI(env, napi_get_cb_info(env, info, &argc, argv, NULL, NULL));
    if (argc < 2) { napi_throw_type_error(env, NULL, "uploadLevels(handle, levels)"); return NULL; }
    handle_t *h = block_handle(env, argv[0], *(void **)&p_upload_levels, "nb_upload_levels"); if (!h) return NULL;
    uint8_t *lv;
    if (!get_levels(env, argv[1], h, &lv)) return NULL;
    int rc = p_upload_levels(h->sim, lv);
    if (rc != NB_OK) return throw_nb(env, rc, h->sim, "nb_upload_levels");
    return undefined(env);
}

static napi_value init_module(napi_env env, napi_value exports)
{
    static const struct { const char *name; napi_callback fn; } fns[] = {
        {"load", js_load}, {"deviceCount", js_device_count}, {"create", js_create}, {"upload", js_upload},
        {"setParams", js_set_params}, {"step", js_step}, {"download", js_download}, {"sync", js_sync},
        {"destroy", js_destroy}, {"enableTiming", js_enable_timing}, {"kernelTimes", js_kernel_times},
        {"variant", js_variant}, {"diagnostics", js_diagnostics}, {"stepTimes", js_step_times},
        {"collectiveInfo", js_collective_info}, {"requestFrame", js_request_frame}, {"frame", js_frame}, {"planQuery", js_plan_query},
        {"fieldEval", js_field_eval}, {"downloadJerk", js_download_jerk}, {"uploadDerivs", js_upload_derivs},
        {"setBlockSteps", js_set_block_steps}, {"blockStats", js_block_stats}, {"downloadLevels", js_download_levels},
        {"uploadLevels", js_upload_levels}, {"neighbors", js_neighbors},
    };
    for (size_t i = 0; i < sizeof fns / sizeof fns[0]; ++i) {
        napi_value f;
        if (napi_create_function(env, fns[i].name, NAPI_AUTO_LENGTH, fns[i].fn, NULL, &f) != napi_ok) return NULL;
        if (napi_set_named_property(env, exports, fns[i].name, f) != napi_ok) return NULL;
    }
    return exports;
}

NAPI_MODULE(nb_napi, init_module)
```

nbody3d-webgpu_amd/nbody3d_amd/capi.py:

```python
import ctypes as C
import os

import numpy as np

_PKG = os.path.dirname(os.path.abspath(__file__))
_LIB_PATH = os.environ.get("NB_ENGINE_LIB") or os.path.normpath(os.path.join(_PKG, "..", "csrc", "libnbody3d_hip.so"))

NB_F32, NB_F64 = 0, 1
NB_FLAG_EXT_STREAM = 1
NB_FLAG_LDS_ONLY = 4
NB_FLAG_NO_FUSE = 8
NB_FLAG_POISON = 16
NB_FLAG_JPK_FENCED = 32
NB_FLAG_NO_SYM = 64
NB_FLAG_SYM_SHARD = 128
NB_FLAG_WHOLE_SWEEPS = 256
NB_FLAG_SINGLE_SWEEPS = 512
NB_RCCL_ID_BYTES = 128
NB_RCCL_OVERLAP = 1
NB_MULTI_PEER, NB_MULTI_RCCL, NB_MULTI_PEER_OVERLAP = 0, 1, 2
NB_NOT_READY = 7
NB_FIELD_AT_BODIES, NB_FIELD_F64, NB_FIELD_DEVICE = 1, 2, 4
NB_NBR_AT_BODIES, NB_NBR_DEVICE = 1, 4
NB_NBR_NONE = 0xffffffff
NB_INT_LEAPFROG, NB_INT_HERMITE4 = 0, 1
INTEGRATORS = {"leapfrog": NB_INT_LEAPFROG, "hermite4": NB_INT_HERMITE4}
STATUS = {0: "NB_OK", 1: "NB_ERR_INVALID", 2: "NB_ERR_NO_DEVICE", 3: "NB_ERR_HIP",
          4: "NB_ERR_STATE", 5: "NB_ERR_NOMEM", 6: "NB_ERR_COMM", 7: "NB_NOT_READY"}
ABI_VERSION = 2
ABI_MINOR = 3


class NBodyError(RuntimeError):
    def __init__(self, code, msg):
        super().__init__("%s: %s" % (STATUS.get(code, code), msg))
        self.code = code


class nb_config(C.Structure):
    _fields_ = [
        ("struct_size", C.c_uint32), ("n", C.c_uint32), ("precision", C.c_uint32), ("tile", C.c_uint32),
        ("eps2", C.c_double), ("device", C.c_int32), ("shard_begin", C.c_uint32), ("shard_count", C.c_uint32),
        ("ext_stream", C.c_void_p), ("ext_bodies", C.c_void_p),
        ("force_variant", C.c_uint32), ("jsplit", C.c_uint32), ("flags", C.c_uint32), ("layer_budget_mib", C.c_uint32),
        ("integrator", C.c_uint32), ("reserved", C.c_uint32 * 3),
    ]


class nb_plan_info(C.Structure):
    _fields_ = [("struct_size", C.c_uint32)] + [(k, C.c_uint32) for k in (
        "kind", "ipl", "ls", "x", "jsplit", "j_per_split", "own_split0", "own_splits",
        "sym", "symw", "sym_rank", "sym_np", "sym_layers", "sym_g0", "sym_g1")] + [
        ("sym_plan", C.c_uint32 * 11), ("tab_len", C.c_uint32), ("variant", C.c_char * 112),
        ("sym_ups", C.c_uint32), ("sym_spill_rows", C.c_uint32), ("sym_rank_plan", C.c_uint32 * 16),
        ("sym_pass", C.c_uint32), ("sym_passes", C.c_uint32), ("sym_pass_k_lo", C.c_uint32), ("sym_pass_k_hi", C.c_uint32),
        ("sym_pass_d0", C.c_uint32), ("sym_local", C.c_uint32)]


class nb_step_timing(C.Structure):
    _fields_ = [("struct_size", C.c_uint32), ("launches", C.c_uint32), ("force_ms", C.c_double), ("sym_reduce_ms", C.c_double),
                ("reduce_scatter_ms", C.c_double), ("integrate_ms", C.c_double), ("allgather_ms", C.c_double),
                ("span_ms", C.c_double), ("reduce_scatters", C.c_uint32), ("allgathers", C.c_uint32)]


class nb_field_request(C.Structure):
    _fields_ = [("struct_size", C.c_uint32), ("m", C.c_uint32), ("flags", C.c_uint32), ("first_body", C.c_uint32),
                ("points", C.c_void_p), ("accel", C.c_void_p), ("phi", C.c_void_p)]


class nb_neighbor_request(C.Structure):
    _fields_ = [("struct_size", C.c_uint32), ("m", C.c_uint32), ("flags", C.c_uint32), ("first_body", C.c_uint32),
                ("points", C.c_void_p), ("radii", C.c_void_p), ("radius", C.c_double),
                ("index", C.c_void_p), ("dist2", C.c_void_p), ("count", C.c_void_p)]


NB_BLOCK_FROZEN = 1


class nb_block_steps(C.Structure):
    _fields_ = [("struct_size", C.c_uint32), ("max_level", C.c_uint32), ("min_level", C.c_uint32), ("flags", C.c_uint32),
                ("eta", C.c_double)]


class nb_block_stats(C.Structure):
    _fields_ = [("struct_size", C.c_uint32), ("enabled", C.c_uint32), ("outer_steps", C.c_uint64), ("block_steps", C.c_uint64),
                ("body_steps", C.c_uint64), ("clamped", C.c_uint64), ("finest_level", C.c_uint32), ("reserved", C.c_uint32)]


EXCHANGE_FN = C.CFUNCTYPE(C.c_int, C.c_void_p, C.c_void_p, C.c_size_t, C.c_uint32, C.c_uint32, C.c_uint32, C.c_void_p)
EXCHANGE_WAIT_FN = C.CFUNCTYPE(C.c_int, C.c_void_p, C.c_void_p)

SYMBOLS = ["nb_abi_version", "nb_device_count", "nb_create", "nb_destroy", "nb_upload", "nb_set_params", "nb_step",
           "nb_download", "nb_sync", "nb_last_error", "nb_device_ptr", "nb_set_exchange",
           "nb_set_exchange_overlapped", "nb_enable_timing",
           "nb_kernel_times", "nb_variant_name", "nb_diagnostics",
           "nb_multi_create", "nb_multi_destroy", "nb_multi_upload", "nb_multi_set_params", "nb_multi_step",
           "nb_multi_download", "nb_multi_sync", "nb_multi_last_error", "nb_multi_variant_name",
           "nb_multi_diagnostics", "nb_multi_set_collective", "nb_multi_collective_info",
           "nb_rccl_unique_id", "nb_rccl_attach", "nb_rccl_detach", "nb_rccl_info",
           "nb_step_times", "nb_step_times2", "nb_integrate_pass", "nb_force_pass", "nb_frame_request", "nb_frame_acquire", "nb_shape_info", "nb_plan_query",
           "nb_abi_minor", "nb_field_eval", "nb_multi_field_eval", "nb_download_jerk", "nb_upload_derivs",
           "nb_set_block_steps", "nb_block_stats", "nb_download_levels", "nb_upload_levels",
           "nb_neighbors", "nb_multi_neighbors", "nb_neighbors_shape"]

_lib = None


def library_path():
    return _LIB_PATH


def load_library():
    global _lib
    if _lib is not None:
        return _lib
    if not os.path.exists(_LIB_PATH):
        raise NBodyError(3, "HIP engine not built: %s is missing (run __graft_entry__.build() or "
                            "make -C nbody3d-webgpu_amd/csrc)" % _LIB_PATH)
    L = C.CDLL(_LIB_PATH)
    vp = C.c_void_p
    L.nb_abi_version.restype = C.c_uint32
    L.nb_abi_minor.restype = C.c_uint32
    L.nb_device_count.restype = C.c_int
    L.nb_create.argtypes = [C.POINTER(nb_config), C.POINTER(vp)]
    L.nb_destroy.argtypes = [vp]
    L.nb_destroy.restype = None
    L.nb_upload.argtypes = [vp, vp, vp, vp]
    L.nb_set_params.argtypes = [vp, C.c_double, C.c_double]
    L.nb_step.argtypes = [vp, C.c_uint32]
    L.nb_download.argtypes = [vp, vp, vp, vp]
    L.nb_sync.argtypes = [vp]
    L.nb_last_error.argtypes = [vp]
    L.nb_last_error.restype = C.c_char_p
    L.nb_device_ptr.argtypes = [vp, C.c_int, C.POINTER(vp)]
    L.nb_set_exchange.argtypes = [vp, EXCHANGE_FN, vp]
    L.nb_set_exchange_overlapped.argtypes = [vp, EXCHANGE_FN, EXCHANGE_WAIT_FN, vp]
    L.nb_enable_timing.argtypes = [vp, C.c_int]
    L.nb_kernel_times.argtypes = [vp, C.POINTER(C.c_double), C.POINTER(C.c_double), C.POINTER(C.c_uint32)]
    L.nb_variant_name.argtypes = [vp]
    L.nb_variant_name.restype = C.c_char_p
    L.nb_diagnostics.argtypes = [vp, C.POINTER(C.c_double)]
    L.nb_multi_create.argtypes = [C.POINTER(nb_config), C.c_uint32, C.POINTER(C.c_int32), C.POINTER(vp)]
    L.nb_multi_destroy.argtypes = [vp]
    L.nb_multi_destroy.restype = None
    L.nb_multi_upload.argtypes = [vp, vp, vp, vp]
    L.nb_multi_set_params.argtypes = [vp, C.c_double, C.c_double]
    L.nb_multi_step.argtypes = [vp, C.c_uint32]
    L.nb_multi_download.argtypes = [vp, vp, vp, vp]
    L.nb_multi_sync.argtypes = [vp]
    L.nb_multi_last_error.argtypes = [vp]
    L.nb_multi_last_error.restype = C.c_char_p
    L.nb_multi_variant_name.argtypes = [vp]
    L.nb_multi_variant_name.restype = C.c_char_p
    L.nb_multi_diagnostics.argtypes = [vp, C.POINTER(C.c_double)]
    L.nb_multi_set_collective.argtypes = [vp, C.c_int]
    L.nb_multi_collective_info.argtypes = [vp, C.POINTER(C.c_int), C.POINTER(C.c_int), C.POINTER(C.c_int)]
    L.nb_rccl_unique_id.argtypes = [vp]
    L.nb_rccl_attach.argtypes = [vp, vp, C.c_int, C.c_int, C.c_uint32]
    L.nb_rccl_detach.argtypes = [vp]
    L.nb_rccl_info.argtypes = [vp, C.POINTER(C.c_int), C.POINTER(C.c_int), C.POINTER(C.c_int)]
    L.nb_step_times.argtypes = [vp, C.POINTER(C.c_double), C.POINTER(C.c_double), C.POINTER(C.c_double),
                                C.POINTER(C.c_uint32)]
    L.nb_step_times2.argtypes = [vp, C.POINTER(nb_step_timing)]
    L.nb_integrate_pass.argtypes = [vp, C.c_uint32, C.POINTER(C.c_double)]
    L.nb_force_pass.argtypes = [vp, C.c_uint32, C.POINTER(C.c_double)]
    L.nb_shape_info.argtypes = [vp] + [C.POINTER(C.c_uint32)] * 4
    L.nb_plan_query.argtypes = [C.POINTER(nb_config), C.c_int, C.c_double, C.POINTER(nb_plan_info), C.POINTER(C.c_uint32), C.c_uint32]
    L.nb_frame_request.argtypes = [vp]
    L.nb_frame_acquire.argtypes = [vp, C.c_int, C.POINTER(C.POINTER(C.c_float)), C.POINTER(C.POINTER(C.c_float)),
                                   C.POINTER(C.c_uint64)]
    if L.nb_abi_minor() >= 4:
        L.nb_field_eval.argtypes = [vp, C.POINTER(nb_field_request)]
        L.nb_multi_field_eval.argtypes = [vp, C.POINTER(nb_field_request)]
    if hasattr(L, "nb_download_jerk"):
        L.nb_download_jerk.argtypes = [vp, vp]
        L.nb_upload_derivs.argtypes = [vp, vp, vp]
    if hasattr(L, "nb_set_block_steps"):
        L.nb_set_block_steps.argtypes = [vp, C.POINTER(nb_block_steps)]
        L.nb_block_stats.argtypes = [vp, C.POINTER(nb_block_stats), C.c_int]
        L.nb_download_levels.argtypes = [vp, vp]
        L.nb_upload_levels.argtypes = [vp, vp]
    if hasattr(L, "nb_neighbors"):
        L.nb_neighbors.argtypes = [vp, C.POINTER(nb_neighbor_request)]
        L.nb_multi_neighbors.argtypes = [vp, C.POINTER(nb_neighbor_request)]
        L.nb_neighbors_shape.argtypes = [vp, C.c_uint32] + [C.POINTER(C.c_uint32)] * 3
    _lib = L
    return L


def abi_version():
    return load_library().nb_abi_version()


def abi_minor():
    return load_library().nb_abi_minor()


def device_count():
    return load_library().nb_device_count()


def rccl_unique_id():
    L = load_library()
    buf = C.create_string_buffer(NB_RCCL_ID_BYTES)
    rc = L.nb_rccl_unique_id(buf)
    if rc != 0:
        raise NBodyError(rc, L.nb_last_error(None).decode())
    return buf.raw


def _ptr(a):
    return None if a is None else a.ctypes.data_as(C.c_void_p)


def _field_request(n, dtype, points, bodies, accel, phi, f64):
    if load_library().nb_abi_minor() < 4:
        raise NBodyError(1, "field(): the loaded library is ABI %d.%d; nb_field_eval needs 2.4" % (abi_version(), abi_minor()))
    req = nb_field_request()
    req.struct_size = C.sizeof(nb_field_request)
    pts = None
    if bodies is not None:
        first, count = int(bodies[0]), int(bodies[1])
        if not (0 <= first < 2 ** 32 and 0 <= count < 2 ** 32):
            raise ValueError("field(): bodies=(first, count) out of range")
        req.flags |= NB_FIELD_AT_BODIES
        req.first_body, req.m = first, count
    if points is not None:
        pts = np.asarray(points, dtype=dtype)
        if pts.ndim == 1:
            pts = pts.reshape(-1, 3 if pts.size % 4 else 4)
        if pts.ndim != 2 or pts.shape[1] not in (3, 4):
            raise ValueError("field(): points must have shape (m, 3) or (m, 4)")
        if pts.shape[1] == 3:
            pts = np.concatenate([pts, np.zeros((len(pts), 1), dtype)], axis=1)
        pts = np.ascontiguousarray(pts)
        if bodies is None:
            req.m = len(pts)
        req.points = _ptr(pts) if len(pts) else None
    out_t = np.float64 if (f64 or dtype == np.float64) else np.float32
    if f64:
        req.flags |= NB_FIELD_F64
    a = np.zeros((req.m, 4), out_t) if accel else None
    f = np.zeros((req.m,), out_t) if phi else None
    req.accel = _ptr(a) if a is not None and a.size else None
    req.phi = _ptr(f) if f is not None and f.size else None
    return req, pts, a, f


def _need_neighbors(what):
    if not hasattr(load_library(), "nb_neighbors"):
        raise NBodyError(1, "%s: the loaded library has no nb_neighbors" % what)


def _neighbor_request(dtype, points, bodies, radius, radii):
    _need_neighbors("neighbors()")
    req = nb_neighbor_request()
    req.struct_size = C.sizeof(nb_neighbor_request)
    pts = rad = None
    if bodies is not None:
        first, count = int(bodies[0]), int(bodies[1])
        if not (0 <= first < 2 ** 32 and 0 <= count < 2 ** 32):
            raise ValueError("neighbors(): bodies=(first, count) out of range")
        req.flags |= NB_NBR_AT_BODIES
        req.first_body, req.m = first, count
    if points is not None:
        pts = np.asarray(points, dtype=dtype)
        if pts.ndim == 1:
            pts = pts.reshape(-1, 3 if pts.size % 4 else 4)
# ... 292 lines not shown
            try:
                return int(begin(bodies, esz, n, sb, sc, stream) or 0)
            except Exception:
                import traceback
                traceback.print_exc()
                return -1

        def t_wait(user, stream):
            try:
                return int(wait(stream) or 0)
            except Exception:
                import traceback
                traceback.print_exc()
                return -1

        self._hook = (EXCHANGE_FN(t_begin), EXCHANGE_WAIT_FN(t_wait))
        self._check(self._L.nb_set_exchange_overlapped(self._h, self._hook[0], self._hook[1], None))

    def enable_timing(self, on=True):
        self._check(self._L.nb_enable_timing(self._h, 1 if on else 0))

    def kernel_times(self):
        f, g, c = C.c_double(), C.c_double(), C.c_uint32()
        self._check(self._L.nb_kernel_times(self._h, C.byref(f), C.byref(g), C.byref(c)))
        return f.value, g.value, c.value

    def step_times(self):
        f, g, x, c = C.c_double(), C.c_double(), C.c_double(), C.c_uint32()
        self._check(self._L.nb_step_times(self._h, C.byref(f), C.byref(g), C.byref(x), C.byref(c)))
        return f.value, g.value, x.value, c.value

    def step_breakdown(self):
        t = nb_step_timing()
        t.struct_size = C.sizeof(nb_step_timing)
        self._check(self._L.nb_step_times2(self._h, C.byref(t)))
        return {k: getattr(t, k) for k, _ in nb_step_timing._fields_ if k != "struct_size"}

    def integrate_pass(self, reps):
        ms = C.c_double()
        self._check(self._L.nb_integrate_pass(self._h, int(reps), C.byref(ms)))
        return ms.value

    def force_pass(self, reps):
        ms = C.c_double()
        self._check(self._L.nb_force_pass(self._h, int(reps), C.byref(ms)))
        return ms.value

    def rccl_attach(self, unique_id, nranks, rank, overlap=False):
        if len(unique_id) != NB_RCCL_ID_BYTES:
            raise ValueError("unique_id must be %d bytes" % NB_RCCL_ID_BYTES)
        buf = C.create_string_buffer(bytes(unique_id), NB_RCCL_ID_BYTES)
        self._check(self._L.nb_rccl_attach(self._h, buf, int(nranks), int(rank), NB_RCCL_OVERLAP if overlap else 0))

    def rccl_detach(self):
        self._check(self._L.nb_rccl_detach(self._h))

    def rccl_info(self):
        a, b, c = C.c_int(), C.c_int(), C.c_int()
        self._check(self._L.nb_rccl_info(self._h, C.byref(a), C.byref(b), C.byref(c)))
        return a.value, b.value, c.value

    def request_frame(self):
        self._check(self._L.nb_frame_request(self._h))

    def frame(self, wait=True):
        pb, ps, st = C.POINTER(C.c_float)(), C.POINTER(C.c_float)(), C.c_uint64()
        rc = self._L.nb_frame_acquire(self._h, 1 if wait else 0, C.byref(pb), C.byref(ps), C.byref(st))
        if rc == NB_NOT_READY:
            return None
        self._check(rc)
        b = np.ctypeslib.as_array(pb, shape=(self.n, 4))
        sp = np.ctypeslib.as_array(ps, shape=(self.n,))
        return b, sp, st.value

    @property
    def variant(self):
        return self._L.nb_variant_name(self._h).decode()

    def shape_info(self):
        v = [C.c_uint32() for _ in range(4)]
        self._check(self._L.nb_shape_info(self._h, *[C.byref(x) for x in v]))
        return dict(zip(("jsplit", "j_per_split", "own_split0", "own_splits"), (x.value for x in v)))

    def diagnostics(self):
        out = (C.c_double * 5)()
        self._check(self._L.nb_diagnostics(self._h, out))
        return out[0], out[1], np.array(out[2:5])

    def field(self, points=None, *, bodies=None, accel=True, phi=True, f64=False):
        req, pts, a, f = _field_request(self.n, self.dtype, points, bodies, accel, phi, f64)
        self._check(self._L.nb_field_eval(self._h, C.byref(req)))
        return a, f

    def field_device(self, points_ptr, m, accel_ptr, phi_ptr, *, bodies=None, f64=False):
        if self._L.nb_abi_minor() < 4:
            raise NBodyError(1, "field_device(): the loaded library is ABI %d.%d; nb_field_eval needs 2.4" % (abi_version(), abi_minor()))
        req = nb_field_request()
        req.struct_size = C.sizeof(nb_field_request)
        req.flags = NB_FIELD_DEVICE | (NB_FIELD_F64 if f64 else 0)
        if bodies is not None:
            req.flags |= NB_FIELD_AT_BODIES
            req.first_body, req.m = int(bodies[0]), int(bodies[1])
        else:
            req.m = int(m)
        req.points = points_ptr or None
        req.accel = accel_ptr or None
        req.phi = phi_ptr or None
        self._check(self._L.nb_field_eval(self._h, C.byref(req)))

    def neighbors(self, points=None, *, bodies=None, radius=None, radii=None):
        req, keep, index, dist2, count = _neighbor_request(self.dtype, points, bodies, radius, radii)
        self._check(self._L.nb_neighbors(self._h, C.byref(req)))
        return index, dist2, count

    def neighbors_device(self, points_ptr, m, index_ptr, dist2_ptr, count_ptr=None, *, bodies=None, radius=None, radii_ptr=None):
        _need_neighbors("neighbors_device()")
        req = nb_neighbor_request()
        req.struct_size = C.sizeof(nb_neighbor_request)
        req.flags = NB_NBR_DEVICE
        if bodies is not None:
            req.flags |= NB_NBR_AT_BODIES
            req.first_body, req.m = int(bodies[0]), int(bodies[1])
        else:
            req.m = int(m)
        req.points = points_ptr or None
        req.radii = radii_ptr or None
        req.radius = 0.0 if radius is None else float(radius)
        req.index = index_ptr or None
        req.dist2 = dist2_ptr or None
        req.count = count_ptr or None
        self._check(self._L.nb_neighbors(self._h, C.byref(req)))

    def neighbors_shape(self, m):
        _need_neighbors("neighbors_shape()")
        v = [C.c_uint32() for _ in range(3)]
        self._check(self._L.nb_neighbors_shape(self._h, int(m), *[C.byref(x) for x in v]))
        return dict(zip(("batch", "chunks", "j_per_chunk"), (x.value for x in v)))

    def close_pairs(self, radius):
        index, dist2, _ = self.neighbors(bodies=(0, self.n))
        return mutual_pairs(index, dist2, radius)

    def body_energies(self):
        b, v, _ = self.read(accel=False)
        _, p = self.field(bodies=(0, self.n), accel=False, phi=True)
        m = b[:, 3].astype(np.float64)
        v = v[:, :3].astype(np.float64)
        return 0.5 * m * (v * v).sum(1), m * p.astype(np.float64)

    def energy_drift(self, steps, every):
        ke0, pe0, _ = self.diagnostics()
        e0 = ke0 + pe0
        out, done = [], 0
        while done < steps:
            k = min(int(every), steps - done)
            if k > 1:
                self.simulate(k - 1)
            _, pe_prev, _ = self.diagnostics()
            self.step()
            ke, _, _ = self.diagnostics()
            done += k
            out.append(abs((ke + pe_prev - e0) / e0))
        return out


class MultiSimulation:
# ... 113 lines not shown
```

Before: 6777 billion pair-interactions/s.

## Add equal-mass specialized symmetric force kernels with runtime mass-uniformity detection

```diff
diff --git a/include/nbody3d_hip.h b/include/nbody3d_hip.h
--- a/include/nbody3d_hip.h
+++ b/include/nbody3d_hip.h
@@ -43,6 +43,8 @@
 #define NB_FLAG_WHOLE_SWEEPS 256u
 
 #define NB_FLAG_SINGLE_SWEEPS 512u
+
+#define NB_FLAG_NO_EQM 1024u
 
 typedef enum nb_array { NB_BODIES = 0, NB_VEL = 1, NB_ACCEL = 2, NB_JERK = 3  } nb_array;
 
@@ -148,6 +150,8 @@
 int nb_shape_info(nb_sim *s, uint32_t *jsplit, uint32_t *j_per_split, uint32_t *own_split0,
                   uint32_t *own_splits);
 
+int nb_eqm_info(nb_sim *s, int *eqm);
+
 
 
 int nb_download_jerk(nb_sim *s, void *jerk);
diff --git a/nbody3d-webgpu_amd/csrc/kernels/symmetric.hip.h b/nbody3d-webgpu_amd/csrc/kernels/symmetric.hip.h
--- a/nbody3d-webgpu_amd/csrc/kernels/symmetric.hip.h
+++ b/nbody3d-webgpu_amd/csrc/kernels/symmetric.hip.h
@@ -196,6 +196,14 @@
     }
 }
 
+template <int = 0>
+__device__ __forceinline__ void symw_record_tail_and_gm(const uint32_t* rec_at, const float4* jrows, nb_u4& rec, uint32_t& tail, uint32_t& gm)
+{
+    constexpr int kTailOffset = 4 * 8 + 6 * 4;
+    asm volatile("s_load_dwordx4 %0, %3, 0x0\n\ts_load_dword %1, %4, %6\n\ts_load_dword %2, %5, 0xc\n\ts_waitcnt lgkmcnt(0)"
+                 : "=&s"(rec), "=&s"(tail), "=&s"(gm) : "s"(rec_at), "s"(__builtin_amdgcn_kernarg_segment_ptr()), "s"(jrows), "n"(kTailOffset) : "memory");
+}
+
 __device__ __forceinline__ SymWK symw_plan_words(uint32_t S, uint32_t cps, uint32_t W, uint32_t ups, uint32_t nsb, uint32_t zc, uint32_t r_layer0, uint32_t t_layer0)
 {
     const uint32_t H = (nsb - 1u) >> 1, n_hi = (nsb & 1u) ? 0u : nsb >> 1;
@@ -203,7 +211,7 @@
     return SymWK{(nsb + (zc ? 1u : 0u)) * S, nsb, W, total_hi, total_lo, n_hi, zc, ups, r_layer0, t_layer0};
 }
 
-template <int NG, int J, bool PAIR>
+template <int NG, int J, bool PAIR, bool EQM = false>
 __device__ __forceinline__ void symw_sweeps(const uint32_t* __restrict__ gtab, const float4* __restrict__ bodies, SymRow* __restrict__ partial, SymRow* __restrict__ spill,
                                             SYMW_PLAN_PARAMS, uint32_t* __restrict__ queue, const uint32_t npieces, const uint32_t pieces_off)
 {
@@ -222,10 +230,13 @@
     const uint32_t ups = pl.ups, ush = (uint32_t)__builtin_ctz(ups), ustep = 64u >> ush,
                    tab1 = 2u * (pl.np / S);
     nb_u4 rec;
-    uint32_t tail[1];
-    symw_record_and_tail(gtab + tab1 + 4u * (active ? w : 0u), rec, tail);
+    uint32_t tail[1], gm_bits = 0;
+    if constexpr (EQM) symw_record_tail_and_gm(gtab + tab1 + 4u * (active ? w : 0u), bodies, rec, tail[0], gm_bits);
+    else symw_record_and_tail(gtab + tab1 + 4u * (active ? w : 0u), rec, tail);
     const float eps2 = __builtin_bit_cast(float, tail[0]);
     const nb_f2 e2 = nb_f2{eps2, eps2};
+    const float gm1 = __builtin_bit_cast(float, gm_bits);
+    const nb_f2 gm = nb_f2{gm1, gm1};
     const uint32_t first_lo = pl.n_hi * pl.total_hi, first_z = first_lo + (pl.nsb - pl.n_hi) * pl.total_lo;
     const uint32_t slot = rec.w;
     NB_STAMP_LIGHT(1);
@@ -250,7 +261,8 @@
 #pragma unroll
                 for (int c = 0; c < NG; ++c) {
                     const float4 b0 = ld4(rb + (2 * c) * 64), b1 = ld4(rb + (2 * c + 1) * 64);
-                    xi[c] = nb_f2{b0.x, b1.x}; yi[c] = nb_f2{b0.y, b1.y}; zi[c] = nb_f2{b0.z, b1.z}; mi[c] = nb_f2{b0.w, b1.w};
+                    xi[c] = nb_f2{b0.x, b1.x}; yi[c] = nb_f2{b0.y, b1.y}; zi[c] = nb_f2{b0.z, b1.z};
+                    if constexpr (!EQM) mi[c] = nb_f2{b0.w, b1.w};
                     ax[c] = nb_f2{0, 0}; ay[c] = nb_f2{0, 0}; az[c] = nb_f2{0, 0};
                 }
             }
@@ -316,9 +328,9 @@
 #pragma unroll
                                     for (int c = 0; c < GW; ++c) r[c] = nb_f2{nb_rsq(r[c].x), nb_rsq(r[c].y)};
 #pragma unroll
-                                    for (int c = 0; c < GW; ++c) si[c] = symw_mul(f, tm, r[c]);
-#pragma unroll
-                                    for (int c = 0; c < GW; ++c) sj[c] = mi[c0g + c] * r[c];
+                                    for (int c = 0; c < GW; ++c) si[c] = EQM ? gm * r[c] : symw_mul(f, tm, r[c]);
+#pragma unroll
+                                    for (int c = 0; c < GW; ++c) sj[c] = EQM ? si[c] : mi[c0g + c] * r[c];
 #pragma unroll
                                     for (int c = 0; c < GW; ++c) ax[c0g + c] = __builtin_elementwise_fma(si[c], dx[c], ax[c0g + c]);
 #pragma unroll
@@ -334,7 +346,8 @@
                                 }
                             }
                             tx = nb_f2{wave_rot1(tx.x), wave_rot1(tx.y)}; ty = nb_f2{wave_rot1(ty.x), wave_rot1(ty.y)};
-                            tz = nb_f2{wave_rot1(tz.x), wave_rot1(tz.y)}; tm = nb_f2{wave_rot1(tm.x), wave_rot1(tm.y)};
+                            tz = nb_f2{wave_rot1(tz.x), wave_rot1(tz.y)};
+                            if constexpr (!EQM) tm = nb_f2{wave_rot1(tm.x), wave_rot1(tm.y)};
                             wave_rot1_add(bx0, sx.x); wave_rot1_add(bx1, sx.y); wave_rot1_add(by0, sy.x); wave_rot1_add(by1, sy.y);
                             wave_rot1_add(bz0, sz.x); wave_rot1_add(bz1, sz.y);
                             __builtin_amdgcn_sched_barrier(0);
@@ -385,10 +398,10 @@
 #pragma unroll
                                 for (int c = 0; c < GW; ++c) r[c] = nb_f2{nb_rsq(r[c].x), nb_rsq(r[c].y)};
 #pragma unroll
-                                for (int c = 0; c < GW; ++c) si[c] = pm * r[c];
+                                for (int c = 0; c < GW; ++c) si[c] = EQM ? gm * r[c] : pm * r[c];
                                 if constexpr (BOTH) {
 #pragma unroll
-                                    for (int c = 0; c < GW; ++c) sj[c] = mi[c0g + c] * r[c];
+                                    for (int c = 0; c < GW; ++c) sj[c] = EQM ? si[c] : mi[c0g + c] * r[c];
                                 }
 #pragma unroll
                                 for (int c = 0; c < GW; ++c) ax[c0g + c] = __builtin_elementwise_fma(si[c], dx[c], ax[c0g + c]);
@@ -408,7 +421,8 @@
                         }
 #pragma unroll
                         for (int uu = 0; uu < J; ++uu) {
-                            tx[uu] = wave_rot1(tx[uu]); ty[uu] = wave_rot1(ty[uu]); tz[uu] = wave_rot1(tz[uu]); tm[uu] = wave_rot1(tm[uu]);
+                            tx[uu] = wave_rot1(tx[uu]); ty[uu] = wave_rot1(ty[uu]); tz[uu] = wave_rot1(tz[uu]);
+                            if constexpr (!EQM) tm[uu] = wave_rot1(tm[uu]);
                             if constexpr (BOTH) {
                                 bx[uu] = nb_f2{wave_rot1(bx[uu].x), wave_rot1(bx[uu].y)};
                                 by[uu] = nb_f2{wave_rot1(by[uu].x), wave_rot1(by[uu].y)};
@@ -516,6 +530,29 @@
 void nb_force_symw_pairs(SYMW_KERNEL_PARAMS)
 {
     symw_sweeps<NG, 1, true>(SYMW_KERNEL_ARGS);
+}
+
+template <int NG, int J>
+__global__ __launch_bounds__(256) __attribute__((amdgpu_waves_per_eu(NG >= 4 ? 2 : 4, NG > 4 ? 2 : (NG < 4 ? 8 : 4))))
+void nb_force_symw_eqm(SYMW_KERNEL_PARAMS)
+{
+    symw_sweeps<NG, J, false, true>(SYMW_KERNEL_ARGS);
+}
+template <int NG>
+__global__ __launch_bounds__(256) __attribute__((amdgpu_waves_per_eu(2, NG > 4 ? 2 : 4)))
+void nb_force_symw_pairs_eqm(SYMW_KERNEL_PARAMS)
+{
+    symw_sweeps<NG, 1, true, true>(SYMW_KERNEL_ARGS);
+}
+
+template <int>
+__global__ __launch_bounds__(kBlock) void nb_eqm_check(const float4* __restrict__ bodies, const float4* __restrict__ vel, const float4* __restrict__ acc,
+                                                      const uint32_t n, uint32_t* __restrict__ flag)
+{
+    const uint32_t i = blockIdx.x * kBlock + threadIdx.x;
+    if (i >= n) return;
+    const uint32_t m0 = __builtin_bit_cast(uint32_t, bodies[0].w), m = __builtin_bit_cast(uint32_t, bodies[i].w);
+    if (m != m0 || !(vel[i].w == 0.f) || !(acc[i].w == 0.f)) *flag = 1u;
 }
 
 __device__ __forceinline__ double wave_rot1(double v)
diff --git a/nbody3d-webgpu_amd/csrc/nb_engine.hip b/nbody3d-webgpu_amd/csrc/nb_engine.hip
--- a/nbody3d-webgpu_amd/csrc/nb_engine.hip
+++ b/nbody3d-webgpu_amd/csrc/nb_engine.hip
@@ -116,8 +116,14 @@
     return ipl == 16 ? (const void*)&nb::nb_force_symw_rank<8> : ipl == 8 ? (const void*)&nb::nb_force_symw_rank<4> : nullptr;
 }
 
-const void* kernel_of(bool f64, const Shape& sh, bool single_sweeps = false)
-{
+bool eqm_shape(bool f64, const Shape& sh) { return !f64 && sh.kind == kSym && sh.ls == 1 && sh.x == 3 && (sh.ipl == 8 || sh.ipl == 16); }
+const void* kernel_of(bool f64, const Shape& sh, bool single_sweeps = false, bool eqm = false)
+{
+    if (eqm) {
+        if (!eqm_shape(f64, sh)) return nullptr;
+        if (sh.ipl == 8) return single_sweeps ? (const void*)&nb::nb_force_symw_eqm<4, 1> : (const void*)&nb::nb_force_symw_pairs_eqm<4>;
+        return single_sweeps ? (const void*)&nb::nb_force_symw_eqm<8, 1> : (const void*)&nb::nb_force_symw_pairs_eqm<8>;
+    }
     switch (sh.kind) {
         case kScalar: return f64 ? scalar_kernel<double>(sh.ipl, sh.ls) : scalar_kernel<float>(sh.ipl, sh.ls);
         case kPkLds: return f64 || (sh.ipl & 1) ? nullptr : pk_force_kernel(sh.ipl / 2, sh.ls, sh.x);
@@ -211,6 +217,23 @@
     return NB_OK;
 }
 
+bool eqm_active(const nb_sim* s) { return s->eqm_capable && s->eqm == nb_sim::kEqmYes && !s->xfn && !s->rccl && std::isfinite((float)s->dt); }
+
+int ensure_eqm(nb_sim* s)
+{
+    if (!s->eqm_capable || s->eqm != nb_sim::kEqmUnknown) return NB_OK;
+    const float4 *b = (const float4*)s->bodies[s->cur], *v = (const float4*)s->vel, *a = (const float4*)s->acc;
+    uint32_t n = s->n, found = 1;
+    uint32_t* flag = s->eqm_flag;
+    void* args[] = {&b, &v, &a, &n, &flag};
+    NB_HIP(s, hipMemsetAsync(flag, 0, sizeof(uint32_t), s->stream));
+    NB_HIP(s, hipLaunchKernel((const void*)&nb::nb_eqm_check<0>, dim3(ceil_div(n, nb::kBlock)), dim3(nb::kBlock), args, 0, s->stream));
+    NB_HIP(s, hipMemcpyAsync(&found, flag, sizeof found, hipMemcpyDeviceToHost, s->stream));
+    NB_HIP(s, hipStreamSynchronize(s->stream));
+    s->eqm = found ? nb_sim::kEqmNo : nb_sim::kEqmYes;
+    return NB_OK;
+}
+
 void launch_kernel(const void* fn, dim3 grid, dim3 block, void** args, hipStream_t stream, hipEvent_t t0, hipEvent_t t1)
 {
     if (t0 || t1) (void)hipExtLaunchKernel(fn, grid, block, args, 0, stream, t0, t1, 0);
@@ -253,7 +276,7 @@
         void* sp = s->sym_spill;
         uint32_t* queue = s->sym_queue;
         uint32_t npieces = s->sym_pieces, pieces_off = 2u * (pl.np / ipb_of(sh)) + 4u * pl.W;
-        if (npieces) (void)hipMemsetAsync(queue, 0, sizeof(uint32_t), s->stream);
+        if (npieces) { const hipError_t e = hipMemsetAsync(queue, 0, sizeof(uint32_t), s->stream); if (e != hipSuccess) s->force_err = e; }
         if (s->f64) {
             double G = s->G, e2 = s->eps2;
             void* args[] = {&tab, &b, &p, &sp, &pl.W, &pl.ups, &pl.nsb, &pl.zc, &pl.r_layer0, &pl.t_layer0, &G, &e2, &queue, &npieces, &pieces_off};
@@ -261,7 +284,7 @@
         } else {
             float e2 = (float)s->eps2;
             void* args[] = {&tab, &b, &p, &sp, &pl.W, &pl.ups, &pl.nsb, &pl.zc, &pl.r_layer0, &pl.t_layer0, &e2, &queue, &npieces, &pieces_off};
-            launch_kernel(kernel_of(false, sh, s->single_sweeps), dim3(ceil_div(pl.W, 4u)), dim3(256), args, s->stream, t0, t1);
+            launch_kernel(kernel_of(false, sh, s->single_sweeps, eqm_active(s)), dim3(ceil_div(pl.W, 4u)), dim3(256), args, s->stream, t0, t1);
         }
         return;
     }
@@ -418,7 +441,7 @@
 bool ensure_graph(nb_sim* s, int which)
 {
     auto& slot = s->graphs[which];
-    if (slot.exec && slot.dt == s->dt && slot.G == s->G && slot.parity == role_parity(s)) return true;
+    if (slot.exec && slot.dt == s->dt && slot.G == s->G && slot.parity == role_parity(s) && slot.eqm == eqm_active(s)) return true;
     if (slot.exec) { (void)hipGraphExecDestroy(slot.exec); slot.exec = nullptr; }
     if (slot.graph) { (void)hipGraphDestroy(slot.graph); slot.graph = nullptr; }
     void *acc0 = s->acc, *par0 = s->partial;
@@ -430,10 +453,10 @@
     hipGraph_t g = nullptr;
     const bool ok = hipStreamEndCapture(s->stream, &g) == hipSuccess && g;
     s->acc = acc0; s->partial = par0; s->cur = cur0; s->acc_parity = par_bit0;
-    if (!ok) { (void)hipGetLastError(); s->graphs_ok = false; return false; }
+    if (!ok || s->force_err != hipSuccess) { if (g) (void)hipGraphDestroy(g); (void)hipGetLastError(); s->force_err = hipSuccess; s->graphs_ok = false; return false; }
     hipGraphExec_t ge = nullptr;
     if (hipGraphInstantiate(&ge, g, nullptr, nullptr, 0) != hipSuccess) { (void)hipGraphDestroy(g); (void)hipGetLastError(); s->graphs_ok = false; return false; }
-    slot.graph = g; slot.exec = ge; slot.dt = s->dt; slot.G = s->G; slot.parity = role_parity(s);
+    slot.graph = g; slot.exec = ge; slot.dt = s->dt; slot.G = s->G; slot.parity = role_parity(s); slot.eqm = eqm_active(s);
     return true;
 }
 
@@ -848,6 +871,8 @@
     }
     if (!kernel_of(s->f64, shape_of(s))) return bail(NB_ERR_INVALID, "nb_create: no kernel for shape " + s->variant);
     s->single_sweeps = (cfg.flags & NB_FLAG_SINGLE_SWEEPS) != 0;
+    s->eqm_capable = !(cfg.flags & NB_FLAG_NO_EQM) && s->symw && !s->sym_rank && cfg.shard_count == 0 && !cfg.ext_bodies && s->sym_np == s->n
+                     && eqm_shape(s->f64, shape_of(s));
 
     const size_t row = 4 * s->esz;
     if (cfg.ext_bodies) { s->bodies[0] = cfg.ext_bodies; s->own_bodies = false; }
@@ -876,6 +901,7 @@
             NB_HIPC(hipMalloc((void**)&s->sym_queue, 64));
             NB_HIPC(hipMemset(s->sym_queue, 0, 64));
         }
+        if (s->eqm_capable) NB_HIPC(hipMalloc((void**)&s->eqm_flag, 64));
         if (s->symw) {
             NB_HIPC(hipMalloc((void**)&s->sym_tab, sizeof(uint32_t) * s->sym_tab_host.size()));
             NB_HIPC(hipMemcpy(s->sym_tab, s->sym_tab_host.data(), sizeof(uint32_t) * s->sym_tab_host.size(), hipMemcpyHostToDevice));
@@ -934,6 +960,7 @@
     if (s->sym_tab) (void)hipFree(s->sym_tab);
     if (s->sym_spill) (void)hipFree(s->sym_spill);
     if (s->sym_queue) (void)hipFree(s->sym_queue);
+    if (s->eqm_flag) (void)hipFree(s->eqm_flag);
     if (s->sym_A) (void)hipFree(s->sym_A);
     for (void* p : {s->jerk, s->hx, s->hv, s->fj_part, (void*)s->blk_lev, (void*)s->blk_due, (void*)s->blk_act, (void*)s->blk_hdr}) if (p) (void)hipFree(p);
     if (s->blk_hdr_host) (void)hipHostFree(s->blk_hdr_host);
@@ -971,6 +998,18 @@
     s->uploaded = true;
     s->pairs_ok = false;
     s->gm_ok = false;
+    if (s->eqm_capable) {
+        const float *hb = (const float*)bodies, *hv = (const float*)vel, *ha = (const float*)accel;
+        uint32_t m0;
+        memcpy(&m0, hb + 3, sizeof m0);
+        bool same = true;
+        for (uint32_t i = 0; i < s->n && same; ++i) {
+            uint32_t m;
+            memcpy(&m, hb + 4 * (size_t)i + 3, sizeof m);
+            same = m == m0 && hv[4 * (size_t)i + 3] == 0.f && (!ha || ha[4 * (size_t)i + 3] == 0.f);
+        }
+        s->eqm = same ? nb_sim::kEqmYes : nb_sim::kEqmNo;
+    }
     return NB_OK;
 }
 
@@ -995,6 +1034,7 @@
     ensure_pairs(s);
     if (gm_active(s) && !s->gm_ok) { if (int rc = finish_gather(s)) return rc; }
     if (int rc = ensure_gm(s)) return rc;
+    if (int rc = ensure_eqm(s)) return rc;
     if (s->own_stream && s->graphs_ok && !exchange && !s->timing && !s->sym_rank && nsteps >= kGraphChunk) {
         for (int which = 1; which >= 0; --which) {
             while (nsteps >= kGraphSteps[which] && ensure_graph(s, which)) {
@@ -1051,6 +1091,7 @@
             else launch_integrate<float>(s, e ? e[6] : nullptr, e ? e[2] : nullptr);
         }
         NB_HIP(s, hipGetLastError());
+        if (s->force_err != hipSuccess) { const hipError_t queue_reset = s->force_err; s->force_err = hipSuccess; NB_HIP(s, queue_reset); }
         ++s->steps_done;
         if (exchange) s->gm_ok = false;
         if (s->rccl) {
@@ -1109,9 +1150,9 @@
         if (int rc = ensure_derivs(s, "nb_device_ptr")) return rc;
     }
     switch (which) {
-        case NB_BODIES: *out = s->bodies[s->cur]; s->pairs_ok = false; s->gm_ok = false; s->derivs_ok = false; s->levels = 0; break;
-        case NB_VEL: *out = s->vel; s->derivs_ok = false; s->levels = 0; break;
-        case NB_ACCEL: *out = s->acc; break;
+        case NB_BODIES: *out = s->bodies[s->cur]; s->pairs_ok = false; s->gm_ok = false; s->derivs_ok = false; s->levels = 0; s->eqm = nb_sim::kEqmUnknown; break;
+        case NB_VEL: *out = s->vel; s->derivs_ok = false; s->levels = 0; s->eqm = nb_sim::kEqmUnknown; break;
+        case NB_ACCEL: *out = s->acc; s->eqm = nb_sim::kEqmUnknown; break;
         case NB_JERK: *out = s->jerk; break;
         default: return fail(s, NB_ERR_INVALID, "nb_device_ptr: unknown array");
     }
@@ -1384,6 +1425,7 @@
     NB_HIP(s, hipSetDevice(s->device));
     if (int rc = finish_gather(s)) return rc;
     if (int rc = ensure_gm(s)) return rc;
+    if (int rc = ensure_eqm(s)) return rc;
     if (s->hermite && !s->params_set) return fail(s, NB_ERR_STATE, "nb_force_pass: nb_set_params has not been called (G)");
     auto once = [&]() -> int {
         if (s->hermite) { launch_fj(s, s->bodies[0], s->vel, s->hx, s->hv); return NB_OK; }
@@ -1403,6 +1445,7 @@
     NB_HIP(s, hipEventElapsedTime(&ms, e0, e1));
     (void)hipEventDestroy(e0); (void)hipEventDestroy(e1);
     NB_HIP(s, hipGetLastError());
+    if (s->force_err != hipSuccess) { const hipError_t queue_reset = s->force_err; s->force_err = hipSuccess; NB_HIP(s, queue_reset); }
     *avg_ms = ms / reps;
     return NB_OK;
 }
@@ -1416,6 +1459,17 @@
     if (j_per_split) *j_per_split = s->j_per_split;
     if (own_split0) *own_split0 = s->own_split0;
     if (own_splits) *own_splits = s->own_splits;
+    return NB_OK;
+}
+
+int nb_eqm_info(nb_sim* s, int* eqm)
+{
+    if (!s || !eqm) return NB_ERR_INVALID;
+    *eqm = 0;
+    if (!s->eqm_capable || !s->uploaded) return NB_OK;
+    NB_HIP(s, hipSetDevice(s->device));
+    if (int rc = ensure_eqm(s)) return rc;
+    *eqm = eqm_active(s) ? 1 : 0;
     return NB_OK;
 }
 
diff --git a/nbody3d-webgpu_amd/csrc/nb_internal.h b/nbody3d-webgpu_amd/csrc/nb_internal.h
--- a/nbody3d-webgpu_amd/csrc/nb_internal.h
+++ b/nbody3d-webgpu_amd/csrc/nb_internal.h
@@ -78,6 +78,11 @@
     uint32_t sym_pieces = 0;
     bool single_sweeps = false;
     uint32_t* sym_queue = nullptr;
+    bool eqm_capable = false;
+    enum { kEqmUnknown = 0, kEqmYes = 1, kEqmNo = 2 };
+    int eqm = kEqmUnknown;
+    uint32_t* eqm_flag = nullptr;
+    hipError_t force_err = hipSuccess;
     bool sym_rank = false;
     uint32_t sym_g0 = 0, sym_g1 = 0;
     uint32_t sym_rank_plan[16] = {0};
@@ -98,6 +103,7 @@
         hipGraphExec_t exec = nullptr;
         double dt = 0.0, G = 0.0;
         int parity = 0;
+        bool eqm = false;
     } graphs[2];
     bool graphs_ok = true;
     std::vector<nb_events> pool;
diff --git a/nbody3d-webgpu_amd/js/addon/nb_napi.c b/nbody3d-webgpu_amd/js/addon/nb_napi.c
--- a/nbody3d-webgpu_amd/js/addon/nb_napi.c
+++ b/nbody3d-webgpu_amd/js/addon/nb_napi.c
@@ -52,6 +52,7 @@
 static int (*p_upload_levels)(nb_sim *, const uint8_t *);
 static int (*p_neighbors)(nb_sim *, const nb_neighbor_request *);
 static int (*p_multi_neighbors)(nb_multi *, const nb_neighbor_request *);
+static int (*p_eqm_info)(nb_sim *, int *);
 
 typedef struct { nb_sim *sim; nb_multi *multi; uint32_t n; int f64; } handle_t;
 
@@ -135,6 +136,7 @@
         *(void **)(&p_upload_levels) = dlsym(h, "nb_upload_levels");
         *(void **)(&p_neighbors) = dlsym(h, "nb_neighbors");
         *(void **)(&p_multi_neighbors) = dlsym(h, "nb_multi_neighbors");
+        *(void **)(&p_eqm_info) = dlsym(h, "nb_eqm_info");
         g_lib = h;
     }
     if (p_abi_version() != NB_ABI_VERSION) { napi_throw_error(env, "NB_ABI", "ABI version mismatch"); return NULL; }
@@ -444,6 +446,21 @@
     return v;
 }
 
+static napi_value js_eqm(napi_env env, napi_callback_info info)
+{
+    size_t argc = 1; napi_value argv[1];
+    CHECK_NAPI(env, napi_get_cb_info(env, info, &argc, argv, NULL, NULL));
+    handle_t *h = argc ? get_handle(env, argv[0]) : NULL; if (!h) return NULL;
+    int eqm = 0;
+    if (h->sim && p_eqm_info) {
+        int rc = p_eqm_info(h->sim, &eqm);
+        if (rc != NB_OK) return throw_nb(env, rc, h->sim, "nb_eqm_info");
+    }
+    napi_value v;
+    CHECK_NAPI(env, napi_get_boolean(env, eqm != 0, &v));
+    return v;
+}
+
 static napi_value js_diagnostics(napi_env env, napi_callback_info info)
 {
     size_t argc = 1; napi_value argv[1];
@@ -781,7 +798,7 @@
         {"load", js_load}, {"deviceCount", js_device_count}, {"create", js_create}, {"upload", js_upload},
         {"setParams", js_set_params}, {"step", js_step}, {"download", js_download}, {"sync", js_sync},
         {"destroy", js_destroy}, {"enableTiming", js_enable_timing}, {"kernelTimes", js_kernel_times},
-        {"variant", js_variant}, {"diagnostics", js_diagnostics}, {"stepTimes", js_step_times},
+        {"variant", js_variant}, {"eqm", js_eqm}, {"diagnostics", js_diagnostics}, {"stepTimes", js_step_times},
         {"collectiveInfo", js_collective_info}, {"requestFrame", js_request_frame}, {"frame", js_frame}, {"planQuery", js_plan_query},
         {"fieldEval", js_field_eval}, {"downloadJerk", js_download_jerk}, {"uploadDerivs", js_upload_derivs},
         {"setBlockSteps", js_set_block_steps}, {"blockStats", js_block_stats}, {"downloadLevels", js_download_levels},
diff --git a/nbody3d-webgpu_amd/nbody3d_amd/capi.py b/nbody3d-webgpu_amd/nbody3d_amd/capi.py
--- a/nbody3d-webgpu_amd/nbody3d_amd/capi.py
+++ b/nbody3d-webgpu_amd/nbody3d_amd/capi.py
@@ -16,6 +16,7 @@
 NB_FLAG_SYM_SHARD = 128
 NB_FLAG_WHOLE_SWEEPS = 256
 NB_FLAG_SINGLE_SWEEPS = 512
+NB_FLAG_NO_EQM = 1024
 NB_RCCL_ID_BYTES = 128
 NB_RCCL_OVERLAP = 1
 NB_MULTI_PEER, NB_MULTI_RCCL, NB_MULTI_PEER_OVERLAP = 0, 1, 2
@@ -101,7 +102,7 @@
            "nb_step_times", "nb_step_times2", "nb_integrate_pass", "nb_force_pass", "nb_frame_request", "nb_frame_acquire", "nb_shape_info", "nb_plan_query",
            "nb_abi_minor", "nb_field_eval", "nb_multi_field_eval", "nb_download_jerk", "nb_upload_derivs",
            "nb_set_block_steps", "nb_block_stats", "nb_download_levels", "nb_upload_levels",
-           "nb_neighbors", "nb_multi_neighbors", "nb_neighbors_shape"]
+           "nb_neighbors", "nb_multi_neighbors", "nb_neighbors_shape", "nb_eqm_info"]
 
 _lib = None
 
@@ -184,6 +185,8 @@
         L.nb_neighbors.argtypes = [vp, C.POINTER(nb_neighbor_request)]
         L.nb_multi_neighbors.argtypes = [vp, C.POINTER(nb_neighbor_request)]
         L.nb_neighbors_shape.argtypes = [vp, C.c_uint32] + [C.POINTER(C.c_uint32)] * 3
+    if hasattr(L, "nb_eqm_info"):
+        L.nb_eqm_info.argtypes = [vp, C.POINTER(C.c_int)]
     _lib = L
     return L
 
@@ -642,6 +645,14 @@
         self._check(self._L.nb_shape_info(self._h, *[C.byref(x) for x in v]))
         return dict(zip(("jsplit", "j_per_split", "own_split0", "own_splits"), (x.value for x in v)))
 
+    @property
+    def eqm(self):
+        if not hasattr(self._L, "nb_eqm_info"):
+            return False
+        v = C.c_int()
+        self._check(self._L.nb_eqm_info(self._h, C.byref(v)))
+        return bool(v.value)
+
     def diagnostics(self):
         out = (C.c_double * 5)()
         self._check(self._L.nb_diagnostics(self._h, out))
```

Measured after the change: 7120 billion pair-interactions/s, median of 6. 5.1% higher.
